# awsaf49/vip-cup-2022

Measured on AMD Instinct MI355X. Metric: images/sec (200x200, full ensemble), higher is better.
Workload: dtype f16; 1 GPU; ensemble8; precision=fast, distinct_images=5120, global_batch=256, parallelism=image-parallel dp1, one all-gather of scores, member_streams=3

## Files before the change

### include/vipcup_hip.h

```cpp
#ifndef VIPCUP_HIP_H
#define VIPCUP_HIP_H

#include <stddef.h>
#include <stdint.h>

#ifdef __cplusplus
extern "C" {
#endif

typedef enum vip_status {
    VIP_OK = 0,
    VIP_ERR_BAD_ARG = -1,
    VIP_ERR_ALIGNMENT = -2,
    VIP_ERR_UNSUPPORTED = -3,
    VIP_ERR_LAUNCH = -4,
    VIP_ERR_JPEG = -5,
    VIP_ERR_PNG = -6,
    VIP_ERR_WEBP = -7
} vip_status;

enum { VIP_ACT_NONE = 0, VIP_ACT_RELU = 1, VIP_ACT_SILU = 2, VIP_ACT_GELU = 3, VIP_ACT_SIGMOID = 4 };

int vip_version(void);
const char* vip_last_error(void);

typedef struct vip_conv_desc {
    int B, H, W;
    int Cin, Cout;
    int kh, kw, sh, sw;
    int pt, pl;
    int Ho, Wo;
    int groups;
    int ldx, cin_off;
    int ldy, cout_off;
    int ldr, res_off;
    int ldw;
    int act_pre, act_post;
} vip_conv_desc;

int vip_conv2d_nhwc_f16(const void* x, const void* w, const float* bias, const void* residual,
                        void* y, const vip_conv_desc* d, void* stream);

int vip_conv2d_gated_nhwc_f16(const void* x, const void* gate, const void* w, const float* bias, const void* residual,
                              void* y, const vip_conv_desc* d, void* stream);

int vip_conv2d_hilo_nhwc_f16(const void* x, const void* w_hi, const void* w_lo, const float* bias, const void* residual,
                             void* y, const vip_conv_desc* d, void* stream);

int vip_conv2d_out_gated_nhwc_f16(const void* x, const void* w, const void* w_lo, const float* bias, const void* out_gate,
                                  const void* residual, void* y, const vip_conv_desc* d, void* stream);
int vip_conv2d_out_gated_variant(const vip_conv_desc* d, int has_w_lo, char* variant, size_t cap);
int vip_conv2d_out_gated2_nhwc_f16(const void* x, const void* w, const void* w_lo, const float* bias, const void* out_gate,
                                   const void* residual, void* y, void* y2, int act2, const vip_conv_desc* d, void* stream);
int vip_conv2d_out_gated2_variant(const vip_conv_desc* d, int has_w_lo, int act2, char* variant, size_t cap);

int vip_gemm_bias_act_f16(const void* A, const void* W, const float* bias, const void* residual,
                          void* C, int M, int N, int K, int lda, int ldw, int ldc, int ldr,
                          int act_pre, int act_post, void* stream);

int vip_ln_gemm_supported(int M, int K, int N, int act);
int vip_ln_gemm_bias_act_f16(const void* A, const float* ln_gamma, const float* ln_beta, float ln_eps, const void* W,
                             const float* bias, const void* residual, void* C, int M, int N, int K, int lda, int ldw,
                             int ldc, int ldr, int act_pre, int act_post, void* stream);

int vip_gemm_split_f16(const void* A, const void* W, const float* bias, void* C, int M, int N, int K, int lda,
                       int ldw, int act, void* stream);

int vip_gemm_split2_f16(const void* A, const void* W, const float* bias, void* C, int M, int N, int K, int ldw, int act,
                        void* stream);
int vip_gemm_split2_hilo_f16(const void* A, const void* W, const void* W_lo, const float* bias, void* C, int M, int N, int K, int ldw,
                             int act, void* stream);

int vip_mlp_fused_supported(int M, int C, int hidden, int act);
int vip_mlp_fused_plan(int M, int C, int hidden, int act, int* workgroups, int* tile_rows);
int vip_mlp_fused_f16(const void* x, const float* ln_gamma, const float* ln_beta, float ln_eps, const void* w1,
                      const float* b1, const void* w2, const float* b2, const void* residual, void* y, int M, int C,
                      int hidden, int ldx, int ldw1, int ldw2, int ldy, int ldr, int act, void* stream);

int vip_se_gate_f16(const void* x, const void* w1, const float* b1, const void* w2, const float* b2, void* gate,
                    int B, int HW, int C, int ldx, int Cr, int ldw1, int Cout, int ldw2, int act1, int act2,
                    int split, void* stream);
int vip_se_gate_hilo_f16(const void* x, const void* w1, const void* w1_lo, const float* b1, const void* w2, const float* b2, void* gate,
                         int B, int HW, int C, int ldx, int Cr, int ldw1, int Cout, int ldw2, int act1, int act2, int split,
                         void* stream);

int vip_dwconv2d_nhwc_f16(const void* x, const float* w, const float* bias, void* y,
                          int B, int H, int W, int C, int k, int stride, int pt, int pl,
                          int Ho, int Wo, int act, void* stream);

int vip_dwconv2d_pool_parts(int B, int H, int W, int C, int k, int stride, int Ho, int Wo);
long vip_dwconv2d_tile_plan(int B, int H, int W, int C, int k, int stride, int Ho, int Wo, int pooled, int* workgroups, int* geom);
int vip_dwconv2d_pool_nhwc_f16(const void* x, const float* w, const float* bias, void* y, float* partials, int parts,
                               int B, int H, int W, int C, int k, int stride, int pt, int pl, int Ho, int Wo, int act,
                               void* stream);
int vip_se_gate_pooled_f16(const float* partials, int parts, const void* w1, const float* b1, const void* w2,
                           const float* b2, void* gate, int B, int HW, int C, int Cr, int ldw1, int Cout, int ldw2,
                           int act1, int act2, int split, void* stream);

int vip_layernorm_f16(const void* x, const float* gamma, const float* beta, void* y,
                      int rows, int C, float eps, void* stream);

int vip_pool2d_nhwc_f16(const void* x, void* y, int B, int H, int W, int C, int ldx, int ldy,
                        int k, int stride, int pt, int pl, int Ho, int Wo, int mode, void* stream);

int vip_global_avgpool_f16(const void* x, void* y, int B, int HW, int C, int ldx, void* stream);

int vip_global_avgpool_split_f16(const void* x, void* y, int B, int HW, int C, int ldx, void* stream);

int vip_gap_dense_f32(const void* x, const float* W, const float* bias, float* out, int B, int HW, int C,
                      int ldx, int N, void* stream);

int vip_gap_ln_dense_f32(const void* x, const float* gamma, const float* beta, float eps, const float* W, const float* bias,
                         float* out, int B, int HW, int C, int ldx, int N, void* stream);

int vip_scale_add_act_f16(const void* x, const void* scale, const void* residual, void* y,
                          int B, int HW, int C, int act, void* stream);
int vip_scale_add_act2_f16(const void* x, const void* scale, const void* residual, void* y, void* y2,
                           int B, int HW, int C, int act, int act2, void* stream);
int vip_scale_add_act3_f16(const void* x, const void* scale, int scale_planes, const void* residual, void* y, void* y2,
                           int B, int HW, int C, int act, int act2, void* stream);

int vip_mul_f16(const void* a, const void* b, void* y, long rows, int C, int lda, int a_off, int ldb, int b_off,
                int ldy, int y_off, void* stream);

int vip_radix_combine_f16(const void* x, const void* scale, void* y, int B, int HW, int C, int radix,
                          void* stream);
int vip_radix_combine2_f16(const void* x, const void* scale, int scale_planes, void* y, int B, int HW, int C, int radix,
                           void* stream);

int vip_gcvit_attn_block_supported(int C, int heads, int ws);
int vip_gcvit_attn_block_f16(const void* x, const void* q_global, const float* ln_gamma, const float* ln_beta, float ln_eps,
                             const void* wqkv, int ldwq, const float* bqkv, const void* wproj, int ldwp, const float* bproj,
                             const float* table, void* y, int B, int Hp, int Wp, int C, int heads, int ws, float scale,
                             void* stream);

int vip_window_attn_fwd_f16(const void* qkv, const void* q_global, const float* bias_table,
                            void* out, int B, int Hp, int Wp, int C, int heads, int ws, int nq,
                            float scale, void* stream);

int vip_mhsa_fwd_f16(const void* qkv, void* out, int B, int N, int D, int heads, float scale,
                     void* stream);

int vip_vit_tokens_f16(const void* patches, const void* cls_token, const void* pos_embed, void* out,
                       int B, int n_patches, int D, void* stream);

typedef struct vip_jpeg_desc {
// ... 357 lines not shown
```

### vip-cup-2022_amd/_abi.py

```python
import ctypes as C
import os

import torch

_HERE = os.path.dirname(os.path.abspath(__file__))
LIB_PATH = os.environ.get("VIP_LIB_PATH") or os.path.join(_HERE, "libvipcup_hip.so")

_lib = None


class VipError(RuntimeError):
    pass


class ConvDesc(C.Structure):
    _fields_ = [(n, C.c_int) for n in (
        "B", "H", "W", "Cin", "Cout", "kh", "kw", "sh", "sw", "pt", "pl", "Ho", "Wo", "groups",
        "ldx", "cin_off", "ldy", "cout_off", "ldr", "res_off", "ldw", "act_pre", "act_post")]


class JpegDesc(C.Structure):
    _fields_ = [("width", C.c_int32), ("height", C.c_int32), ("ncomp", C.c_int32),
                ("hsamp", C.c_int32 * 3), ("vsamp", C.c_int32 * 3),
                ("blocks_w", C.c_int32 * 3), ("blocks_h", C.c_int32 * 3),
                ("coef_off", C.c_int64 * 3), ("qt", (C.c_uint16 * 64) * 3), ("rgb_coded", C.c_int32)]


class PngDesc(C.Structure):
    _fields_ = [("width", C.c_int32), ("height", C.c_int32), ("bit_depth", C.c_int32), ("color_type", C.c_int32),
                ("interlace", C.c_int32), ("channels", C.c_int32), ("bpp", C.c_int32), ("palette_size", C.c_int32),
                ("stream_off", C.c_int64), ("pass_off", C.c_int64 * 7), ("pass_w", C.c_int32 * 7), ("pass_h", C.c_int32 * 7),
                ("palette", (C.c_uint8 * 3) * 256)]


class WebpDesc(C.Structure):
    _fields_ = [("width", C.c_int32), ("height", C.c_int32), ("has_alpha", C.c_int32), ("coded_width", C.c_int32),
                ("n_transforms", C.c_int32), ("stats", C.c_int32), ("type", C.c_int32 * 4), ("bits", C.c_int32 * 4),
                ("xsize", C.c_int32 * 4), ("stream_off", C.c_int64), ("data_off", C.c_int64 * 4), ("argb_off", C.c_int64)]


class Vp8Mb(C.Structure):
    _fields_ = [("ymode", C.c_uint8), ("uvmode", C.c_uint8), ("flevel", C.c_uint8), ("ilevel", C.c_uint8), ("hev", C.c_uint8),
                ("inner", C.c_uint8), ("segment", C.c_uint8), ("skip", C.c_uint8), ("bmodes", C.c_uint8 * 16), ("nz", C.c_uint32),
                ("dc_only", C.c_uint32), ("coef_idx", C.c_uint32), ("reserved", C.c_uint32)]


class Vp8Desc(C.Structure):
    _fields_ = [("width", C.c_int32), ("height", C.c_int32), ("mb_w", C.c_int32), ("mb_h", C.c_int32), ("has_alpha", C.c_int32),
                ("filter_type", C.c_int32), ("stats", C.c_int64), ("stream_off", C.c_int64), ("mb_off", C.c_int64),
                ("coef_off", C.c_int64), ("coef_blocks", C.c_int64), ("plane_off", C.c_int64)]


class Vp8EncParams(C.Structure):
    _fields_ = [("quality", C.c_int32), ("base_q", C.c_int32), ("y1", C.c_int32 * 2), ("y2", C.c_int32 * 2), ("uv", C.c_int32 * 2),
                ("filter_level", C.c_int32), ("flevel", C.c_int32), ("ilevel", C.c_int32), ("hev", C.c_int32), ("i4_bias", C.c_int32),
                ("reserved", C.c_int32), ("y1_inv", C.c_uint32 * 2), ("y2_inv", C.c_uint32 * 2), ("uv_inv", C.c_uint32 * 2)]


_vp, _i, _f, _sz = C.c_void_p, C.c_int, C.c_float, C.c_size_t

SIGNATURES = {
    "vip_version": (_i, []),
    "vip_last_error": (C.c_char_p, []),
    "vip_conv2d_nhwc_f16": (_i, [_vp, _vp, _vp, _vp, _vp, C.POINTER(ConvDesc), _vp]),
    "vip_conv2d_gated_nhwc_f16": (_i, [_vp, _vp, _vp, _vp, _vp, _vp, C.POINTER(ConvDesc), _vp]),
    "vip_conv2d_hilo_nhwc_f16": (_i, [_vp, _vp, _vp, _vp, _vp, _vp, C.POINTER(ConvDesc), _vp]),
    "vip_conv2d_out_gated_nhwc_f16": (_i, [_vp, _vp, _vp, _vp, _vp, _vp, _vp, C.POINTER(ConvDesc), _vp]),
    "vip_conv2d_out_gated_variant": (_i, [C.POINTER(ConvDesc), _i, C.c_char_p, _sz]),
    "vip_conv2d_out_gated2_nhwc_f16": (_i, [_vp, _vp, _vp, _vp, _vp, _vp, _vp, _vp, _i, C.POINTER(ConvDesc), _vp]),
    "vip_conv2d_out_gated2_variant": (_i, [C.POINTER(ConvDesc), _i, _i, C.c_char_p, _sz]),
    "vip_gemm_bias_act_f16": (_i, [_vp, _vp, _vp, _vp, _vp] + [_i] * 9 + [_vp]),
    "vip_ln_gemm_supported": (_i, [_i, _i, _i, _i]),
    "vip_ln_gemm_bias_act_f16": (_i, [_vp, _vp, _vp, _f] + [_vp] * 4 + [_i] * 9 + [_vp]),
    "vip_mlp_fused_supported": (_i, [_i, _i, _i, _i]),
    "vip_mlp_fused_plan": (_i, [_i] * 4 + [C.POINTER(_i)] * 2),
    "vip_mlp_fused_f16": (_i, [_vp, _vp, _vp, _f] + [_vp] * 6 + [_i] * 9 + [_vp]),
    "vip_se_gate_f16": (_i, [_vp] * 6 + [_i] * 11 + [_vp]),
    "vip_se_gate_hilo_f16": (_i, [_vp] * 7 + [_i] * 11 + [_vp]),
    "vip_gemm_split_f16": (_i, [_vp, _vp, _vp, _vp] + [_i] * 6 + [_vp]),
    "vip_gemm_split2_f16": (_i, [_vp, _vp, _vp, _vp] + [_i] * 5 + [_vp]),
    "vip_gemm_split2_hilo_f16": (_i, [_vp, _vp, _vp, _vp, _vp] + [_i] * 5 + [_vp]),
    "vip_dwconv2d_nhwc_f16": (_i, [_vp, _vp, _vp, _vp] + [_i] * 11 + [_vp]),
    "vip_dwconv2d_pool_parts": (_i, [_i] * 8),
    "vip_dwconv2d_tile_plan": (C.c_long, [_i] * 9 + [C.POINTER(_i)] * 2),
    "vip_dwconv2d_pool_nhwc_f16": (_i, [_vp, _vp, _vp, _vp, _vp] + [_i] * 12 + [_vp]),
    "vip_se_gate_pooled_f16": (_i, [_vp, _i] + [_vp] * 5 + [_i] * 10 + [_vp]),
    "vip_layernorm_f16": (_i, [_vp, _vp, _vp, _vp, _i, _i, _f, _vp]),
    "vip_pool2d_nhwc_f16": (_i, [_vp, _vp] + [_i] * 13 + [_vp]),
    "vip_global_avgpool_f16": (_i, [_vp, _vp, _i, _i, _i, _i, _vp]),
    "vip_global_avgpool_split_f16": (_i, [_vp, _vp, _i, _i, _i, _i, _vp]),
    "vip_gap_dense_f32": (_i, [_vp, _vp, _vp, _vp, _i, _i, _i, _i, _i, _vp]),
    "vip_experiments_built": (_i, []),
    "vip_gcvit_attn_block_supported": (_i, [_i, _i, _i]),
    "vip_gcvit_attn_block_f16": (_i, [_vp, _vp, _vp, _vp, _f, _vp, _i, _vp, _vp, _i, _vp, _vp, _vp] + [_i] * 6 + [_f, _vp]),
    "vip_mbconv_expand_dw_supported": (_i, [_i, _i, _i, _i]),
    "vip_mbconv_expand_dw_f16": (_i, [_vp] * 7 + [_i] * 14 + [_vp]),
    "vip_head_prob_f32": (_i, [_vp, _vp, _vp, _i, _i, _vp]),
    "vip_head_act_f32": (_i, [_vp, _vp, _i, _i, _i, _vp]),
    "vip_prob_to_score_f32": (_i, [_vp, _vp, _i, _i, _vp]),
    "vip_ensemble_mean_f32": (_i, [_vp, _vp, _i, _i, C.c_long, _vp]),
    "vip_gap_ln_dense_f32": (_i, [_vp, _vp, _vp, _f, _vp, _vp, _vp, _i, _i, _i, _i, _i, _vp]),
    "vip_scale_add_act_f16": (_i, [_vp, _vp, _vp, _vp, _i, _i, _i, _i, _vp]),
    "vip_scale_add_act2_f16": (_i, [_vp, _vp, _vp, _vp, _vp, _i, _i, _i, _i, _i, _vp]),
    "vip_scale_add_act3_f16": (_i, [_vp, _vp, _i, _vp, _vp, _vp, _i, _i, _i, _i, _i, _vp]),
    "vip_mul_f16": (_i, [_vp, _vp, _vp, C.c_long] + [_i] * 7 + [_vp]),
    "vip_radix_combine_f16": (_i, [_vp, _vp, _vp, _i, _i, _i, _i, _vp]),
    "vip_radix_combine2_f16": (_i, [_vp, _vp, _i, _vp, _i, _i, _i, _i, _vp]),
    "vip_window_attn_fwd_f16": (_i, [_vp, _vp, _vp, _vp] + [_i] * 7 + [_f, _vp]),
    "vip_mhsa_fwd_f16": (_i, [_vp, _vp, _i, _i, _i, _i, _f, _vp]),
    "vip_jpeg_probe_h": (_i, [_vp, _sz, _vp, _vp]),
    "vip_jpeg_entropy_decode_h": (_i, [_vp, _vp, _i, _vp, _vp, _sz, _vp, _i]),
    "vip_jpeg_idct_rgb_u8": (_i, [_vp, _vp, _i, _i, _vp, _vp, _i, _i, _vp]),
    "vip_jpeg_quality_tables_h": (_i, [_i, _vp, _vp]),
    "vip_jpeg_encode_layout_h": (_i, [_i, _i, _i, _i, _vp, _vp]),
    "vip_jpeg_fdct_quant_u8": (_i, [_vp, _vp, _i, _i, _vp, _vp, _i, _i, _vp]),
    "vip_resample_coeffs_h": (_i, [_i, _i, _i, _vp, _sz, _vp, _sz, _vp]),
    "vip_resample_tile_shape": (_i, [_vp, _vp, _vp]),
    "vip_resample_rgb_u8": (_i, [_vp, _vp, _i, _i, _vp, _vp, _i, _i, _vp, _vp, _i, _i, _i, _vp]),
    "vip_blur_weights_h": (_i, [C.c_double, _i, _vp, _sz]),
    "vip_blur_gauss_rgb_u8": (_i, [_vp, _vp, _i, _i, _vp, _i, _i, _vp, _i, _i, _vp]),
    "vip_median_rgb_u8": (_i, [_vp, _vp, _i, _i, _vp, _i, _i, _i, _i, _vp]),
    "vip_sharpen_rgb_u8": (_i, [_vp, _vp, _i, _i, _vp, _i, _i, _vp, _i, _i, _i, _i, _vp]),
    "vip_warp_affine_rgb_u8": (_i, [_vp, _vp, _i, _i, _vp, _vp, _i, _i, _vp, _i, _i, _vp]),
    "vip_colour_rgb_u8": (_i, [_vp, _vp, _i, _i, _vp, _i, _i, _vp, _vp, _vp, _i, _vp]),
    "vip_noise_rgb_u8": (_i, [_vp, _vp, _i, _i, _vp, _i, _i, _i, C.c_int64, C.c_uint32, _vp, _vp, _i, _vp]),
    "vip_noise_rgb_u8_placed": (_i, [_vp, _vp, _i, _i, _vp, _i, _i, _i, C.c_int64, C.c_uint32, _vp, _vp, _i, _i, _vp]),
    "vip_tone_hist_u8": (_i, [_vp, _vp, _i, _i, _i, _i, _i, _vp, _i, _vp]),
    "vip_tone_lut_u8": (_i, [_vp, _i, _i, _i, _i, _vp, _vp]),
    "vip_tone_apply_rgb_u8": (_i, [_vp, _vp, _i, _i, _vp, _i, _i, _vp, _i, _i, _i, _i, _vp]),
    "vip_tone_apply_rgb_u8_placed": (_i, [_vp, _vp, _i, _i, _vp, _i, _i, _vp, _i, _i, _i, _i, _i, _vp]),
    "vip_png_probe_h": (_i, [_vp, _sz, _vp, _vp]),
    "vip_png_inflate_h": (_i, [_vp, _vp, _i, _vp, _vp, _sz, _vp, _i]),
    "vip_png_unfilter_rgb_u8": (_i, [_vp, _vp, _i, _vp, _i, _i, _vp]),
    "vip_webp_probe_h": (_i, [_vp, _sz, _vp, _vp]),
    "vip_webp_entropy_h": (_i, [_vp, _vp, _i, _vp, _vp, _sz, _vp, _i]),
    "vip_webp_inverse_rgb_u8": (_i, [_vp, _vp, _i, _vp, _i, _i, _vp]),
    "vip_vp8_probe_h": (_i, [_vp, _sz, _vp, _vp]),
    "vip_vp8_entropy_h": (_i, [_vp, _vp, _i, _vp, _vp, _sz, _vp, _i]),
    "vip_vp8_scratch_bytes": (_i, [_vp, _i, _vp]),
    "vip_vp8_reconstruct_rgb_u8": (_i, [_vp, _sz, _vp, _i, _vp, _sz, _vp, _i, _i, _vp]),
    "vip_vp8_default_stages": (_i, []),
    "vip_vp8_reconstruct_stages_rgb_u8": (_i, [_vp, _sz, _vp, _i, _vp, _sz, _vp, _i, _i, _i, _vp]),
    "vip_vp8_encode_params_h": (_i, [_i, _vp]),
    "vip_vp8_encode_layout_h": (_i, [_vp, _i, _i, _vp, _vp, _vp]),
    "vip_vp8_encode_rgb_u8": (_i, [_vp, _vp, _i, _i, _i, _i, _vp, _sz, _vp, _sz, _vp, _sz, _vp]),
    "vip_bicubic_table_f32": (_i, [_vp]),
    "vip_resize_bicubic_norm_f16": (_i, [_vp, _vp, _vp, _i, _i, _i, _vp, _i, _i, _i, _vp]),
    "vip_tile_resize_bicubic_norm_f16": (_i, [_vp, _vp, _vp, _i, _i, _i, _i, _vp, _i, _i, _i, _vp]),
    "vip_tile_resize_bicubic_norm_s32": (_i, [_vp, _vp, _vp, _i, _i, _i, _i, _vp, _i, _i, _i, _vp]),
    "vip_tile_aggregate_f32": (_i, [_vp, _vp, _i, _i, _i, _f, _vp, _vp]),
    "vip_image_mean_u8": (_i, [_vp, _vp, _i, _i, _i, _vp, _vp]),
    "vip_occlude_resize_bicubic_norm_f16": (_i, [_vp] * 5 + [_i] * 4 + [_vp, _i, _i, _i, _vp]),
    "vip_occlude_resize_bicubic_norm_s32": (_i, [_vp] * 5 + [_i] * 4 + [_vp, _i, _i, _i, _vp]),
    "vip_occlusion_cells_f32": (_i, [_vp, _vp, _vp, _i, _i, _i, _i, _i, _f, _vp, _vp, _vp]),
    "vip_occlusion_map": (_i, [_vp, _vp, _i, _i, _i, _i, _vp, _i, _vp]),
    "vip_tta_augment_f16": (_i, [_vp, _vp, _vp, _i, _i, _i, _i, _vp]),
# ... 81 lines not shown
```

### vip-cup-2022_amd/csrc/conv_igemm.hip

```cpp
#include "common.hpp"
#include <stdlib.h>
#include <string.h>
#include <type_traits>

#ifndef VIP_GEMM_H2
#define VIP_GEMM_H2 0
#endif

#ifndef VIP_MFMA_PRIO
#define VIP_MFMA_PRIO 1
#endif
#ifndef VIP_MFMA_PRIO_TILE
#define VIP_MFMA_PRIO_TILE 1
#endif

namespace {

constexpr bool H2 = VIP_GEMM_H2;
__device__ __forceinline__ int h2_pos(int c) { return H2 ? (((c & 1) << 2) | (c >> 1)) : c; }
constexpr unsigned OOB2 = 0xFFFFFFE0u;
constexpr int ESZ = H2 ? 4 : 2;

struct ConvArgs {
    const f16* x;
    const f16* w;
    const float* bias;
    const f16* res;
    f16* y;
    int H, W, Ho, Wo;
    int Cin_g, Cout_g;
    int kh, kw, sh, sw, pt, pl;
    int ldx, ldy, ldr, ldw;
    int cin_off, cout_off, res_off;
    int M, K;
    long x_span_bytes;
    long y_span_bytes, res_span_bytes;
    int bias_elems;
    int act_pre, act_post;
    int m_blocks, n_blocks;
    const f16* w_lo;
    const f16* gate;
    int y_lo_off;
    int gate_hw;
    const f16* ogate;
    int ogate_elems;
    unsigned hw_magic;
    float out_scale;
    int* status;
    const float* ln_g;
    const float* ln_b;
    float ln_eps;
};

struct ConvArgs2 : ConvArgs {
    f16* y2;
};

enum Family { PW_GEMM, ROWS_GEMM, GEMM8P, PWX, PWK_DIRECT, PWK_GEMM, IM2COL, CONV_IGEMM };
struct Plan {
    Family family;
    int mode;
    int ng, pt, wn, ks, ksc, bm, bn;
    bool gated, hilo, ln, xsplit, pipe;
    bool pf2;
    int m_blocks, n_blocks;
    int n_chunks, nb_ch, lds_stride;
};

template <int... Vs, class F>
int with_const(int v, F&& f) {
    int st = VIP_ERR_UNSUPPORTED;
    if (!((v == Vs && ((st = f(std::integral_constant<int, Vs>{})), true)) || ...)) vip_set_error("vip_conv2d_nhwc_f16: no instantiation for %d", v);
    return st;
}

inline int device_cus() {
    static const int cus = [] {
        hipDeviceProp_t pr;
        int dev = 0;
        return (hipGetDevice(&dev) == hipSuccess && hipGetDeviceProperties(&pr, dev) == hipSuccess && pr.multiProcessorCount > 0)
                   ? pr.multiProcessorCount : 256;
    }();
    return cus;
}

template <int ACT, bool RES, int POST>
__device__ __forceinline__ void h2_store8(const ConvArgs& a, const f32x4& q0, const f32x4& q1, unsigned off, unsigned roff,
                                          const __amdgpu_buffer_rsrc_t& rb_res, const __amdgpu_buffer_rsrc_t& rb_y) {
    f32x2 p[4] = {{q0[0], q0[1]}, {q0[2], q0[3]}, {q1[0], q1[1]}, {q1[2], q1[3]}};
#pragma unroll
    for (int e = 0; e < 4; ++e) p[e] = vip_act2<ACT>(p[e] * a.out_scale);
    if constexpr (RES) {
        const uint4 rh = __builtin_bit_cast(uint4, __builtin_amdgcn_raw_buffer_load_b128(rb_res, roff, 0, 0));
        const uint4 rl = __builtin_bit_cast(uint4, __builtin_amdgcn_raw_buffer_load_b128(rb_res, roff + 16u, 0, 0));
        const unsigned rhw[4] = {rh.x, rh.y, rh.z, rh.w}, rlw[4] = {rl.x, rl.y, rl.z, rl.w};
#pragma unroll
        for (int e = 0; e < 4; ++e) {
            float px = p[e].x, py = p[e].y;
            asm("v_fma_mix_f32 %0, %1, 1.0, %0 op_sel_hi:[1,0,0]" : "+v"(px) : "v"(rhw[e]));
            asm("v_fma_mix_f32 %0, %1, 1.0, %0 op_sel:[1,0,0] op_sel_hi:[1,0,0]" : "+v"(py) : "v"(rhw[e]));
            asm("v_fma_mix_f32 %0, %1, 1.0, %0 op_sel_hi:[1,0,0]" : "+v"(px) : "v"(rlw[e]));
            asm("v_fma_mix_f32 %0, %1, 1.0, %0 op_sel:[1,0,0] op_sel_hi:[1,0,0]" : "+v"(py) : "v"(rlw[e]));
            p[e] = (f32x2){px, py};
        }
    }
    if constexpr (POST == 1) {
#pragma unroll
        for (int e = 0; e < 4; ++e) p[e] = (f32x2){fmaxf(p[e].x, 0.f), fmaxf(p[e].y, 0.f)};
    } else if constexpr (POST == 2) {
#pragma unroll
        for (int e = 0; e < 4; ++e) p[e] = (f32x2){vip_act_strict(p[e].x, a.act_post), vip_act_strict(p[e].y, a.act_post)};
    }
    typedef unsigned short u16x2 __attribute__((ext_vector_type(2)));
    unsigned hw[4], lw[4];
    u16x2 mx = {0, 0};
#pragma unroll
    for (int e = 0; e < 4; ++e) {
        hw[e] = __builtin_bit_cast(unsigned, __builtin_convertvector(p[e], f16x2));
        const float px = p[e].x, py = p[e].y;
        asm("v_fma_mixlo_f16 %0, %1, -1.0, %2 op_sel_hi:[1,0,0]" : "=v"(lw[e]) : "v"(hw[e]), "v"(px));
        asm("v_fma_mixhi_f16 %0, %1, -1.0, %2 op_sel:[1,0,0] op_sel_hi:[1,0,0]" : "+v"(lw[e]) : "v"(hw[e]), "v"(py));
        mx = __builtin_elementwise_max(mx, __builtin_bit_cast(u16x2, hw[e] & 0x7FFF7FFFu));
    }
    typedef __attribute__((__vector_size__(4 * sizeof(unsigned)))) unsigned u32x4;
    const u32x4 oh = {hw[0], hw[1], hw[2], hw[3]}, ol = {lw[0], lw[1], lw[2], lw[3]};
    __builtin_amdgcn_raw_buffer_store_b128(oh, rb_y, off, 0, 0);
    __builtin_amdgcn_raw_buffer_store_b128(ol, rb_y, off + 16u, 0, 0);
    if (a.status && off != OOB2 && (mx.x >= 0x7C00 || mx.y >= 0x7C00)) *a.status = VIP_H2_OVERFLOW;
}

__device__ __forceinline__ int swz_x(int row, int chunk) { return row * 128 + ((chunk ^ (row & 7)) << 4); }
__device__ __forceinline__ int swz_w(int row, int chunk) {
    const int key = (((row >> 3) & 3) << 1) | ((row >> 1) & 1);
    return row * 128 + ((chunk ^ key) << 4);
}

template <int ACT>
__device__ __forceinline__ float act_t(float v) {
    if constexpr (ACT == VIP_ACT_RELU) return v > 0.f ? v : 0.f;
    else if constexpr (ACT == VIP_ACT_SILU) return v * vip_sigmoid(v);
    else if constexpr (ACT == VIP_ACT_GELU) return 0.5f * v * (1.f + vip_erf(v * 0.70710678118654752f));
    else if constexpr (ACT == VIP_ACT_SIGMOID) return vip_sigmoid(v);
    else return v;
}

template <int MT, int ACT>
__device__ __forceinline__ void epilogue(const ConvArgs& a, f32x4 (&acc)[MT][4], int m_base, int n_first, int group) {
// ... 192 lines not shown
        const char* sb = sa + A_BYTES;
#pragma unroll
        for (int ks = 0; ks < 2; ++ks) {
            const int ch = ks * 4 + lq;
            U4H8 wf[4], xf[MT];
#pragma unroll
            for (int nt = 0; nt < 4; ++nt) wf[nt].u = *reinterpret_cast<const uint4*>(sb + swz_w(wrow_base + (nt >> 1) * 32 + (nt & 1) * 4, ch));
#pragma unroll
            for (int mt = 0; mt < MT; ++mt) xf[mt].u = *reinterpret_cast<const uint4*>(sa + swz_x(xrow_base + mt * 16, ch));
            if constexpr (H2) {
                U4H8 wl[4];
                if (ks == 0) {
#pragma unroll
                    for (int nt = 0; nt < 4; ++nt) wl[nt].u = *reinterpret_cast<const uint4*>(sb + swz_w(wrow_base + (nt >> 1) * 32 + (nt & 1) * 4, 4 + lq));
                } else {
#pragma unroll
                    for (int nt = 0; nt < 4; ++nt) wf[nt].u = *reinterpret_cast<const uint4*>(sb + swz_w(wrow_base + (nt >> 1) * 32 + (nt & 1) * 4, lq));
                }
                if (VIP_MFMA_PRIO_TILE) __builtin_amdgcn_s_setprio(1);
#pragma unroll
                for (int mt = 0; mt < MT; ++mt)
#pragma unroll
                    for (int nt = 0; nt < 4; ++nt) {
                        if (ks == 0) acc[mt][nt] = __builtin_amdgcn_mfma_f32_16x16x32_f16(wl[nt].h, xf[mt].h, acc[mt][nt], 0, 0, 0);
                        acc[mt][nt] = __builtin_amdgcn_mfma_f32_16x16x32_f16(wf[nt].h, xf[mt].h, acc[mt][nt], 0, 0, 0);
                    }
                if (VIP_MFMA_PRIO_TILE) __builtin_amdgcn_s_setprio(0);
                continue;
            }
            if (VIP_MFMA_PRIO_TILE) __builtin_amdgcn_s_setprio(1);
#pragma unroll
            for (int mt = 0; mt < MT; ++mt)
#pragma unroll
                for (int nt = 0; nt < 4; ++nt)
                    acc[mt][nt] = __builtin_amdgcn_mfma_f32_16x16x32_f16(wf[nt].h, xf[mt].h, acc[mt][nt], 0, 0, 0);
            if (VIP_MFMA_PRIO_TILE) __builtin_amdgcn_s_setprio(0);
        }
        if (kt + 1 < nk) store_tiles(buf ^ 1);
        __syncthreads();
    }

    const int m_base = m0 + wave_m0 + l15;
    const int n_first = n0 + wave_n0 + lq * 8;
    switch (a.act_pre) {
        case VIP_ACT_RELU: epilogue<MT, VIP_ACT_RELU>(a, acc, m_base, n_first, group); break;
        case VIP_ACT_SILU: epilogue<MT, VIP_ACT_SILU>(a, acc, m_base, n_first, group); break;
        case VIP_ACT_GELU: epilogue<MT, VIP_ACT_GELU>(a, acc, m_base, n_first, group); break;
        case VIP_ACT_SIGMOID: epilogue<MT, VIP_ACT_SIGMOID>(a, acc, m_base, n_first, group); break;
        default: epilogue<MT, VIP_ACT_NONE>(a, acc, m_base, n_first, group); break;
    }
}

struct GateLds {
    const float* g;
    int img0, stride, n0;
};

__device__ __forceinline__ unsigned image_of(const ConvArgs& a, unsigned m) {
    unsigned img = __umulhi(m, a.hw_magic);
    if (m - img * (unsigned)a.gate_hw >= (unsigned)a.gate_hw) ++img;
    return img;
}

__device__ __forceinline__ int stage_out_gate(const ConvArgs& a, float* g_lds, int stride, int m_first, int rows, int n0, int nch, int t,
                                              int nthreads) {
    const __amdgpu_buffer_rsrc_t rb_g = __builtin_amdgcn_make_buffer_rsrc((void*)a.ogate, 0, (unsigned)a.ogate_elems * 2u, 0x00020000);
    const int img0 = (int)image_of(a, (unsigned)min(m_first, a.M - 1)), img1 = (int)image_of(a, (unsigned)min(m_first + rows - 1, a.M - 1));
    const int q = nch >> 2;
    for (int i = t; i < (img1 - img0 + 1) * q; i += nthreads) {
        const int im = i / q, c = (i - im * q) * 4, n = n0 + c;
        const unsigned off = n < a.Cout_g ? ((unsigned)(img0 + im) * 2u * (unsigned)a.Cout_g + (unsigned)n) * 2u : 0xFFFFFFF0u;
        typedef __attribute__((__vector_size__(2 * sizeof(unsigned)))) unsigned u32x2;
        const u32x2 hv = __builtin_amdgcn_raw_buffer_load_b64(rb_g, off, 0, 0);
        const u32x2 lv = __builtin_amdgcn_raw_buffer_load_b64(rb_g, n < a.Cout_g ? off + (unsigned)a.Cout_g * 2u : 0xFFFFFFF0u, 0, 0);
        const f16x4 hh = __builtin_bit_cast(f16x4, hv), ll = __builtin_bit_cast(f16x4, lv);
        f32x4 gv;
#pragma unroll
        for (int j = 0; j < 4; ++j) gv[j] = (float)hh[j] + (float)ll[j];
        *reinterpret_cast<f32x4*>(g_lds + im * stride + c) = gv;
    }
    return img0;
}

template <int PT, int ACT, bool RES, bool POST_RELU, bool OGATE = false, bool Y2 = false>
__device__ __forceinline__ void pw_epilogue(const ConvArgs& a, f32x4 (&acc)[PT][4], int m_base, int n_first,
                                            const __amdgpu_buffer_rsrc_t& rb_res, const __amdgpu_buffer_rsrc_t& rb_y, GateLds gl = GateLds{},
                                            const __amdgpu_buffer_rsrc_t* rb_y2 = nullptr) {
    constexpr unsigned OOB = 0xFFFFFFF0u;
    if constexpr (H2) {
#pragma unroll
        for (int p = 0; p < PT; ++p) {
            const int m = m_base + p * 16;
#pragma unroll
            for (int h = 0; h < 2; ++h) {
                const int n = n_first + h * 32;
                const bool ok = (m < a.M) & (n < a.Cout_g);
                const unsigned off = ok ? (unsigned)(((long)m * a.ldy + a.cout_off + n) * 4) : OOB2;
                const unsigned roff = (RES && ok) ? (unsigned)(((long)m * a.ldr + a.res_off + n) * 4) : OOB2;
                h2_store8<ACT, RES, POST_RELU ? 1 : 0>(a, acc[p][h * 2], acc[p][h * 2 + 1], off, roff, rb_res, rb_y);
            }
        }
        return;
    }
    static_assert(!(OGATE && H2), "the output gate is carried by the fp16-storage build only");
    static_assert(OGATE || !Y2, "the second output belongs to the output-gated epilogue");
#pragma unroll
    for (int p = 0; p < PT; ++p) {
        const int m = m_base + p * 16;
        int g_row = 0;
        if constexpr (OGATE) g_row = m < a.M ? ((int)image_of(a, (unsigned)m) - gl.img0) * gl.stride - gl.n0 : -gl.n0;
#pragma unroll
        for (int h = 0; h < 2; ++h) {
            const int n = n_first + h * 32;
            const bool ok = (m < a.M) & (n < a.Cout_g);
            U4H8 r;
            f32x4 g0, g1;
            if constexpr (RES)
                r.u = __builtin_bit_cast(uint4, __builtin_amdgcn_raw_buffer_load_b128(
                                                    rb_res, ok ? ((unsigned)m * (unsigned)a.ldr + (unsigned)(a.res_off + n)) * 2u : OOB, 0, 0));
            if constexpr (OGATE) {
                g0 = *reinterpret_cast<const f32x4*>(gl.g + g_row + n);
                g1 = *reinterpret_cast<const f32x4*>(gl.g + g_row + n + 4);
            }
            U4H8 o;
#pragma unroll
            for (int j = 0; j < 8; j += 2) {
                const f32x4 av = acc[p][h * 2 + (j >> 2)];
                f32x2 t = vip_act2<ACT>((f32x2){av[j & 3], av[(j & 3) + 1]});
                if constexpr (OGATE) {
                    const f32x4 gq = j < 4 ? g0 : g1;
                    t = t * (f32x2){gq[j & 3], gq[(j & 3) + 1]};
                }
                if constexpr (RES) t = t + (f32x2){(float)r.e[j], (float)r.e[j + 1]};
                if constexpr (POST_RELU) t = (f32x2){fmaxf(t.x, 0.f), fmaxf(t.y, 0.f)};
                o.e[j] = (f16)t.x;
                o.e[j + 1] = (f16)t.y;
            }
            __builtin_amdgcn_raw_buffer_store_b128(
                __builtin_bit_cast(__attribute__((__vector_size__(4 * sizeof(unsigned)))) unsigned, o.u), rb_y,
                ok ? ((unsigned)m * (unsigned)a.ldy + (unsigned)(a.cout_off + n)) * 2u : OOB, 0, 0);
            if constexpr (Y2) {
                U4H8 o2;
#pragma unroll
                for (int j = 0; j < 8; ++j) o2.e[j] = (f16)vip_act((float)o.e[j], VIP_ACT_SILU);
                __builtin_amdgcn_raw_buffer_store_b128(
                    __builtin_bit_cast(__attribute__((__vector_size__(4 * sizeof(unsigned)))) unsigned, o2.u), *rb_y2,
                    ok ? ((unsigned)m * (unsigned)a.ldy + (unsigned)(a.cout_off + n)) * 2u : OOB, 0, 0);
            }
        }
    }
}

template <int KS, int PT, bool PRE, bool HILO, bool OG = false, bool Y2 = false>
__global__ __launch_bounds__(256, 2) void pw_gemm_kernel(std::conditional_t<Y2, ConvArgs2, ConvArgs> a, int nb_ch, int lds_stride, int n_tiles,
                                                         int mode) {
    static_assert(OG || !Y2, "the second output belongs to the output-gated instantiations");
    extern __shared__ __attribute__((aligned(16))) char smem[];
    const int tid = threadIdx.x, lane = tid & 63, wave = tid >> 6;
    const int l15 = lane & 15, lq = lane >> 4;
    const int n_chunk0 = blockIdx.y * nb_ch;
    const int nch = min(nb_ch, ((a.Cout_g - n_chunk0) + 63) & ~63);
    constexpr unsigned OOB = 0xFFFFFFF0u;
    float* bias_lds = reinterpret_cast<float*>(smem + nb_ch * lds_stride);
    constexpr int OG_IMAGES = 4;
    float* g_lds = bias_lds + nb_ch + (tid >> 6) * (OG_IMAGES * nb_ch);

    {
        const __amdgpu_buffer_rsrc_t rw = __builtin_amdgcn_make_buffer_rsrc(
            (void*)a.w, 0, (unsigned)min((long)0xFFFFFFF0L, 2L * a.Cout_g * a.ldw), 0x00020000);
        const __amdgpu_buffer_rsrc_t rwl = __builtin_amdgcn_make_buffer_rsrc(
            (void*)a.w_lo, 0, HILO ? (unsigned)min((long)0xFFFFFFF0L, 2L * a.Cout_g * a.ldw) : 0u, 0x00020000);
        const int cpr = KS * 4;
        constexpr int HALVES = HILO ? 2 : 1;
        for (int i = tid; i < nch * cpr * HALVES; i += 256) {
            const int j = i / (cpr * HALVES), c2 = i - j * (cpr * HALVES);
            const int c = c2 < cpr ? c2 : c2 - cpr;
            const int t = (j >> 4) & 3, r = j & 15;
            const int ch = n_chunk0 + (j & ~63) + (t >> 1) * 32 + (r >> 2) * 8 + (t & 1) * 4 + (r & 3);
            const bool ok = (ch < a.Cout_g) & (c * 8 < a.K);
            const unsigned off = ok ? (unsigned)((ch * a.ldw + c * 8) * 2) : OOB;
            const uint4 v = __builtin_bit_cast(uint4, c2 < cpr ? __builtin_amdgcn_raw_buffer_load_b128(rw, off, 0, 0)
                                                               : __builtin_amdgcn_raw_buffer_load_b128(rwl, off, 0, 0));
            *reinterpret_cast<uint4*>(smem + j * lds_stride + (H2 ? ((c2 & ~7) | h2_pos(c2 & 7)) : c2) * 16) = v;
        }
        const __amdgpu_buffer_rsrc_t rb = __builtin_amdgcn_make_buffer_rsrc(
            (void*)a.bias, 0, a.bias ? (unsigned)(a.bias_elems * 4) : 0u, 0x00020000);
        for (int i = tid; i < nch; i += 256) {
            const int ch = n_chunk0 + i;
            bias_lds[i] = __builtin_bit_cast(float, __builtin_amdgcn_raw_buffer_load_b32(rb, ch < a.Cout_g ? (unsigned)(ch * 4) : OOB, 0, 0));
        }
    }
    __syncthreads();

    const __amdgpu_buffer_rsrc_t rx = __builtin_amdgcn_make_buffer_rsrc(
        (void*)(a.x + a.cin_off), 0, (unsigned)min((long)0xFFFFFFF0L, a.x_span_bytes - 2L * a.cin_off), 0x00020000);
    const __amdgpu_buffer_rsrc_t rb_res =
        __builtin_amdgcn_make_buffer_rsrc((void*)a.res, 0, a.res ? (unsigned)a.res_span_bytes : 0u, 0x00020000);
    const __amdgpu_buffer_rsrc_t rb_y = __builtin_amdgcn_make_buffer_rsrc((void*)a.y, 0, (unsigned)a.y_span_bytes, 0x00020000);
    const char* wl = smem + l15 * lds_stride + lq * 16;

    auto load_x = [&](int tile, U4H8 (&xf)[KS][PT]) {
        const int m0 = tile * (64 * PT) + wave * (16 * PT);
#pragma unroll
        for (int ks = 0; ks < KS; ++ks)
#pragma unroll
            for (int p = 0; p < PT; ++p) {
                const int m = m0 + p * 16 + l15, k = H2 ? (ks >> 1) * 64 + lq * 16 + (ks & 1) * 8 : ks * 32 + lq * 8;
                const bool ok = (m < a.M) & (k < a.K);
                xf[ks][p].u = __builtin_bit_cast(
                    uint4, __builtin_amdgcn_raw_buffer_load_b128(rx, ok ? (unsigned)((m * a.ldx + k) * 2) : OOB, 0, 0));
            }
// ... 56 lines not shown
                for (int p = 0; p < PT; ++p)
#pragma unroll
                    for (int nt = 0; nt < 4; ++nt)
                        acc[p][nt] = __builtin_amdgcn_mfma_f32_16x16x32_f16(wf[nt].h, xf[ks][p].h, ks == 0 ? bv[nt] : acc[p][nt], 0, 0, 0);
                if constexpr (HILO) {
#pragma unroll
                    for (int nt = 0; nt < 4; ++nt) wf[nt].u = *reinterpret_cast<const uint4*>(ws + nt * 16 * lds_stride + (KS + ks) * 64);
#pragma unroll
                    for (int p = 0; p < PT; ++p)
#pragma unroll
                        for (int nt = 0; nt < 4; ++nt)
                            acc[p][nt] = __builtin_amdgcn_mfma_f32_16x16x32_f16(wf[nt].h, xf[ks][p].h, acc[p][nt], 0, 0, 0);
                }
            }
            const int m_base = m0 + l15, n_first = n_chunk0 + sub + lq * 8;
            if constexpr (Y2) {
                const __amdgpu_buffer_rsrc_t rb_y2 = __builtin_amdgcn_make_buffer_rsrc((void*)a.y2, 0, (unsigned)a.y_span_bytes, 0x00020000);
                if (mode == 8) pw_epilogue<PT, VIP_ACT_NONE, true, true, true, true>(a, acc, m_base, n_first, rb_res, rb_y, gl, &rb_y2);
                else pw_epilogue<PT, VIP_ACT_NONE, true, false, true, true>(a, acc, m_base, n_first, rb_res, rb_y, gl, &rb_y2);
            } else if constexpr (OG) {
                if (mode == 8) pw_epilogue<PT, VIP_ACT_NONE, true, true, true>(a, acc, m_base, n_first, rb_res, rb_y, gl);
                else pw_epilogue<PT, VIP_ACT_NONE, true, false, true>(a, acc, m_base, n_first, rb_res, rb_y, gl);
            } else
            switch (mode) {
                case 1: pw_epilogue<PT, VIP_ACT_RELU, false, false>(a, acc, m_base, n_first, rb_res, rb_y); break;
                case 2: pw_epilogue<PT, VIP_ACT_SILU, false, false>(a, acc, m_base, n_first, rb_res, rb_y); break;
                case 3: pw_epilogue<PT, VIP_ACT_GELU, false, false>(a, acc, m_base, n_first, rb_res, rb_y); break;
                case 4: pw_epilogue<PT, VIP_ACT_SIGMOID, false, false>(a, acc, m_base, n_first, rb_res, rb_y); break;
                case 5: pw_epilogue<PT, VIP_ACT_NONE, true, false>(a, acc, m_base, n_first, rb_res, rb_y); break;
                case 6: pw_epilogue<PT, VIP_ACT_NONE, true, true>(a, acc, m_base, n_first, rb_res, rb_y); break;
                default: pw_epilogue<PT, VIP_ACT_NONE, false, false>(a, acc, m_base, n_first, rb_res, rb_y); break;
            }
        }
        if constexpr (PRE) {
#pragma unroll
            for (int ks = 0; ks < KS; ++ks)
#pragma unroll
                for (int p = 0; p < PT; ++p) xf[ks][p] = xn[ks][p];
        } else {
            if (tile + (int)gridDim.x < n_tiles) load_x(tile + gridDim.x, xf);
        }
    }
}

constexpr size_t pw_og_lds(int nb_ch) { return (size_t)4 * 4 * nb_ch * 4; }

template <int KS, int PT, bool HILO, bool OG = false>
int launch_pw(const ConvArgs& a, const Plan& p, hipStream_t s) {
    constexpr bool PRE = OG ? KS <= 2 : KS <= 3;
    const int n_tiles = (a.M + 64 * PT - 1) / (64 * PT);
    int gx = (2 * device_cus() + p.n_chunks - 1) / p.n_chunks;
    if (gx > n_tiles) gx = n_tiles;
    static bool attr_set = false;
    if (!attr_set) {
        (void)hipFuncSetAttribute(reinterpret_cast<const void*>(pw_gemm_kernel<KS, PT, PRE, HILO, OG>),
                                  hipFuncAttributeMaxDynamicSharedMemorySize, 160 * 1024);
        attr_set = true;
    }
    hipLaunchKernelGGL((pw_gemm_kernel<KS, PT, PRE, HILO, OG>), dim3((unsigned)gx, (unsigned)p.n_chunks), dim3(256),
                       (size_t)p.nb_ch * (p.lds_stride + 4) + (OG ? pw_og_lds(p.nb_ch) : 0), s, a, p.nb_ch, p.lds_stride, n_tiles, p.mode);
    return vip_launch_status("vip_conv2d_nhwc_f16(pw)");
}

template <int KS, int PT, bool HILO>
int launch_pw_og2(const ConvArgs& a, const Plan& p, f16* y2, hipStream_t s) {
    constexpr bool PRE = KS <= 2;
    const int n_tiles = (a.M + 64 * PT - 1) / (64 * PT);
    int gx = (2 * device_cus() + p.n_chunks - 1) / p.n_chunks;
    if (gx > n_tiles) gx = n_tiles;
    static bool attr_set = false;
    if (!attr_set) {
        (void)hipFuncSetAttribute(reinterpret_cast<const void*>(pw_gemm_kernel<KS, PT, PRE, HILO, true, true>),
                                  hipFuncAttributeMaxDynamicSharedMemorySize, 160 * 1024);
        attr_set = true;
    }
    ConvArgs2 a2;
    static_cast<ConvArgs&>(a2) = a;
    a2.y2 = y2;
    hipLaunchKernelGGL((pw_gemm_kernel<KS, PT, PRE, HILO, true, true>), dim3((unsigned)gx, (unsigned)p.n_chunks), dim3(256),
                       (size_t)p.nb_ch * (p.lds_stride + 4) + pw_og_lds(p.nb_ch), s, a2, p.nb_ch, p.lds_stride, n_tiles, p.mode);
    return vip_launch_status("vip_conv2d_out_gated2_nhwc_f16(pw)");
}

template <int NG, bool GATED, int PT = 4, bool OG2 = false>
__global__ __launch_bounds__(256, 2) void pwk_direct_kernel(std::conditional_t<OG2, ConvArgs2, ConvArgs> a, int mode) {
    static_assert(!(OG2 && (GATED || H2)), "the second output: fp16 storage, no input gate");
    constexpr int NB = 64 * NG, ROWB = 160;
    constexpr int STAGE = NB * ROWB;
    constexpr int W_IT = NB / 32;
    __shared__ __attribute__((aligned(16))) char smem[2 * STAGE];
    const int tid = threadIdx.x, lane = tid & 63, wave = tid >> 6;
    const int l15 = lane & 15, lq = lane >> 4;
    constexpr unsigned OOB = 0xFFFFFFF0u;

    int bid = blockIdx.x;
    {
        const int nwg = gridDim.x;
        const int q = nwg >> 3, r = nwg & 7;
        const int xcd = bid & 7, idx = bid >> 3;
        bid = (xcd < r ? xcd * (q + 1) : r * (q + 1) + (xcd - r) * q) + idx;
    }
    const int mb = bid / a.n_blocks, nb = bid - mb * a.n_blocks;
    const int m0 = mb * (64 * PT) + wave * (16 * PT);
    const int n0 = nb * NB;

    const __amdgpu_buffer_rsrc_t rw = __builtin_amdgcn_make_buffer_rsrc(
        (void*)a.w, 0, (unsigned)min((long)0xFFFFFFF0L, 2L * a.Cout_g * a.ldw), 0x00020000);
    const __amdgpu_buffer_rsrc_t rx = __builtin_amdgcn_make_buffer_rsrc(
        (void*)(a.x + a.cin_off), 0, (unsigned)min((long)0xFFFFFFF0L, a.x_span_bytes - 2L * a.cin_off), 0x00020000);
    const __amdgpu_buffer_rsrc_t rb_res =
        __builtin_amdgcn_make_buffer_rsrc((void*)a.res, 0, a.res ? (unsigned)a.res_span_bytes : 0u, 0x00020000);
    const __amdgpu_buffer_rsrc_t rb_y = __builtin_amdgcn_make_buffer_rsrc((void*)a.y, 0, (unsigned)a.y_span_bytes, 0x00020000);
    const __amdgpu_buffer_rsrc_t rb_bias =
        __builtin_amdgcn_make_buffer_rsrc((void*)a.bias, 0, a.bias ? (unsigned)(a.bias_elems * 4) : 0u, 0x00020000);

    const int wc = tid & 7;
    unsigned w_off[W_IT];
    int w_lds[W_IT];
#pragma unroll
    for (int i = 0; i < W_IT; ++i) {
        const int j = (tid >> 3) + 32 * i;
        const int t = (j >> 4) & 3, r = j & 15;
        const int ch = n0 + (j & ~63) + (t >> 1) * 32 + (r >> 2) * 8 + (t & 1) * 4 + (r & 3);
        w_off[i] = ch < a.Cout_g ? (unsigned)((ch * a.ldw + wc * 8) * 2) : OOB;
        w_lds[i] = j * ROWB + h2_pos(wc) * 16;
    }
    unsigned x_off[PT];
#pragma unroll
    for (int p = 0; p < PT; ++p) {
        const int m = m0 + p * 16 + l15;
        x_off[p] = m < a.M ? (unsigned)((m * a.ldx + lq * (H2 ? 16 : 8)) * 2) : 0xFFFF0000u;
    }
    const __amdgpu_buffer_rsrc_t rg = __builtin_amdgcn_make_buffer_rsrc(
        (void*)a.gate, 0, GATED ? (unsigned)min((long)0xFFFFFFF0L, (H2 ? 2L : 4L) * ((a.M + a.gate_hw - 1) / a.gate_hw) * a.K) : 0u, 0x00020000);
    unsigned g_off[PT];
#pragma unroll
    for (int p = 0; p < PT; ++p) {
        const int m = m0 + p * 16 + l15;
        g_off[p] = (GATED && m < a.M) ? (H2 ? (unsigned)((m / a.gate_hw) * a.K * 2 + lq * 32) : (unsigned)(((m / a.gate_hw) * 2 * a.K + lq * 8) * 2))
                                      : 0xFFFF0000u;
    }
    const int nk = (a.K + 63) >> 6;

    uint4 wst[W_IT];
    auto load_w = [&](int kc) {
        const bool ok = kc * 64 + wc * 8 < a.K;
#pragma unroll
        for (int i = 0; i < W_IT; ++i)
            wst[i] = __builtin_bit_cast(uint4, __builtin_amdgcn_raw_buffer_load_b128(rw, ok ? w_off[i] + kc * 128 : OOB, 0, 0));
    };
    auto store_w = [&](int buf) {
#pragma unroll
        for (int i = 0; i < W_IT; ++i) *reinterpret_cast<uint4*>(smem + buf * STAGE + w_lds[i]) = wst[i];
    };
    U4H8 xf[2][PT], gq[GATED ? 2 : 1][GATED ? PT : 1];
    auto load_x = [&](int kc, int ks) {
        const bool ok = kc * 64 + (H2 ? lq * 16 + ks * 8 : ks * 32 + lq * 8) < a.K;
#pragma unroll
        for (int p = 0; p < PT; ++p)
            xf[ks][p].u = __builtin_bit_cast(
                uint4, __builtin_amdgcn_raw_buffer_load_b128(rx, ok ? x_off[p] + kc * 128 + ks * (H2 ? 16 : 64) : OOB, 0, 0));
    };
    auto load_g = [&](int kc, int ks) {
        if constexpr (GATED && H2) {
            const bool ok = kc * 64 + lq * 16 < a.K;
#pragma unroll
            for (int p = 0; p < PT; ++p) {
                gq[0][p].u = __builtin_bit_cast(uint4, __builtin_amdgcn_raw_buffer_load_b128(rg, ok ? g_off[p] + kc * 128 : OOB, 0, 0));
                gq[1][p].u = __builtin_bit_cast(uint4, __builtin_amdgcn_raw_buffer_load_b128(rg, ok ? g_off[p] + kc * 128 + 16 : OOB, 0, 0));
            }
        } else if constexpr (GATED) {
            const bool ok = kc * 64 + ks * 32 + lq * 8 < a.K;
#pragma unroll
            for (int p = 0; p < PT; ++p) {
                gq[0][p].u = __builtin_bit_cast(
                    uint4, __builtin_amdgcn_raw_buffer_load_b128(rg, ok ? g_off[p] + kc * 128 + ks * 64 : OOB, 0, 0));
                gq[1][p].u = __builtin_bit_cast(
                    uint4, __builtin_amdgcn_raw_buffer_load_b128(rg, ok ? g_off[p] + kc * 128 + ks * 64 + 2 * a.K : OOB, 0, 0));
            }
        }
    };
    auto gate_x = [&](int ks) {
        if constexpr (GATED && H2) {
#pragma unroll
            for (int p = 0; p < PT; ++p) {
                float xv[8], gv[8];
                h2_join8(xf[0][p], xf[1][p], xv);
                h2_join8(gq[0][p], gq[1][p], gv);
#pragma unroll
                for (int j = 0; j < 8; ++j) xv[j] *= gv[j];
                h2_split8(xv, xf[0][p], xf[1][p]);
            }
        } else if constexpr (GATED) {
#pragma unroll
            for (int p = 0; p < PT; ++p)
                xf[ks][p].h = __builtin_elementwise_fma(xf[ks][p].h, gq[0][p].h, xf[ks][p].h * gq[1][p].h);
        }
    };

    f32x4 acc[NG][PT][4];
    {
#pragma unroll
        for (int g = 0; g < NG; ++g)
#pragma unroll
            for (int nt = 0; nt < 4; ++nt) {
                const int n = n0 + g * 64 + (nt >> 1) * 32 + lq * 8 + (nt & 1) * 4;
                const f32x4 bv = __builtin_bit_cast(
                    f32x4, __builtin_amdgcn_raw_buffer_load_b128(rb_bias, n < a.Cout_g ? (unsigned)(n * 4) : OOB, 0, 0));
#pragma unroll
                for (int p = 0; p < PT; ++p) acc[g][p][nt] = bv;
            }
    }

    load_w(0);
    load_x(0, 0);
    load_x(0, 1);
    load_g(0, 0);
    store_w(0);
    __syncthreads();

    auto compute = [&](int buf, int ks) {
        const char* ws = smem + buf * STAGE + l15 * ROWB + lq * 16 + ks * 64;
#pragma unroll
        for (int g = 0; g < NG; ++g) {
            U4H8 wf[4];
            if constexpr (H2) {
                const char* wh = ws - ks * 64;
                U4H8 wl[4];
#pragma unroll
                for (int nt = 0; nt < 4; ++nt) wf[nt].u = *reinterpret_cast<const uint4*>(wh + (g * 64 + nt * 16) * ROWB);
                if (ks == 0) {
#pragma unroll
                    for (int nt = 0; nt < 4; ++nt) wl[nt].u = *reinterpret_cast<const uint4*>(wh + 64 + (g * 64 + nt * 16) * ROWB);
                }
                if (VIP_MFMA_PRIO) __builtin_amdgcn_s_setprio(1);
#pragma unroll
                for (int nt = 0; nt < 4; ++nt)
#pragma unroll
                    for (int p = 0; p < PT; ++p) {
                        if (ks == 0) acc[g][p][nt] = __builtin_amdgcn_mfma_f32_16x16x32_f16(wl[nt].h, xf[0][p].h, acc[g][p][nt], 0, 0, 0);
                        acc[g][p][nt] = __builtin_amdgcn_mfma_f32_16x16x32_f16(wf[nt].h, xf[ks][p].h, acc[g][p][nt], 0, 0, 0);
                    }
                if (VIP_MFMA_PRIO) __builtin_amdgcn_s_setprio(0);
                continue;
            }
#pragma unroll
            for (int nt = 0; nt < 4; ++nt) wf[nt].u = *reinterpret_cast<const uint4*>(ws + (g * 64 + nt * 16) * ROWB);
            if (VIP_MFMA_PRIO) __builtin_amdgcn_s_setprio(1);
#pragma unroll
            for (int nt = 0; nt < 4; ++nt)
#pragma unroll
                for (int p = 0; p < PT; ++p)
                    acc[g][p][nt] = __builtin_amdgcn_mfma_f32_16x16x32_f16(wf[nt].h, xf[ks][p].h, acc[g][p][nt], 0, 0, 0);
            if (VIP_MFMA_PRIO) __builtin_amdgcn_s_setprio(0);
        }
    };

    for (int kc = 0; kc < nk; ++kc) {
        const int buf = kc & 1;
        load_w(kc + 1);
        __builtin_amdgcn_sched_barrier(0);
        if constexpr (GATED && H2) {
            gate_x(0);
            __builtin_amdgcn_sched_barrier(0);
            load_g(kc + 1, 0);
            __builtin_amdgcn_sched_barrier(0);
        } else if constexpr (GATED) {
            gate_x(0);
            __builtin_amdgcn_sched_barrier(0);
            load_g(kc, 1);
            __builtin_amdgcn_sched_barrier(0);
        }
        compute(buf, 0);
        __builtin_amdgcn_sched_barrier(0);
        load_x(kc + 1, 0);
        __builtin_amdgcn_sched_barrier(0);
        if constexpr (GATED && !H2) {
            gate_x(1);
            __builtin_amdgcn_sched_barrier(0);
            load_g(kc + 1, 0);
            __builtin_amdgcn_sched_barrier(0);
        }
        compute(buf, 1);
        __builtin_amdgcn_sched_barrier(0);
        load_x(kc + 1, 1);
        store_w(buf ^ 1);
        __syncthreads();
    }

    int m_base = m0 + l15, n_lane = n0 + lq * 8;
    asm volatile("" : "+v"(m_base), "+v"(n_lane));
    GateLds gl{};
#if !VIP_GEMM_H2
    if constexpr (!GATED) {
        if (mode >= 7) {
            float* g_lds = reinterpret_cast<float*>(smem);
            const int img0 = stage_out_gate(a, g_lds, NB, mb * (64 * PT), 64 * PT, n0, NB, (int)threadIdx.x, 256);
            __syncthreads();
            gl = GateLds{g_lds, img0, NB, n0};
        }
    }
#endif
    auto epi = [&](auto gtag) {
        constexpr int G_ = decltype(gtag)::value;
        const int n_first = n_lane + G_ * 64;
#if !VIP_GEMM_H2
        if constexpr (OG2) {
            const __amdgpu_buffer_rsrc_t rb_y2 = __builtin_amdgcn_make_buffer_rsrc((void*)a.y2, 0, (unsigned)a.y_span_bytes, 0x00020000);
            if (mode == 8) pw_epilogue<PT, VIP_ACT_NONE, true, true, true, true>(a, acc[G_], m_base, n_first, rb_res, rb_y, gl, &rb_y2);
            else pw_epilogue<PT, VIP_ACT_NONE, true, false, true, true>(a, acc[G_], m_base, n_first, rb_res, rb_y, gl, &rb_y2);
            return;
        }
#endif
        switch (mode) {
            case 1: pw_epilogue<PT, VIP_ACT_RELU, false, false>(a, acc[G_], m_base, n_first, rb_res, rb_y); break;
            case 2: pw_epilogue<PT, VIP_ACT_SILU, false, false>(a, acc[G_], m_base, n_first, rb_res, rb_y); break;
            case 3: pw_epilogue<PT, VIP_ACT_GELU, false, false>(a, acc[G_], m_base, n_first, rb_res, rb_y); break;
            case 4: pw_epilogue<PT, VIP_ACT_SIGMOID, false, false>(a, acc[G_], m_base, n_first, rb_res, rb_y); break;
            case 5: pw_epilogue<PT, VIP_ACT_NONE, true, false>(a, acc[G_], m_base, n_first, rb_res, rb_y); break;
            case 6: pw_epilogue<PT, VIP_ACT_NONE, true, true>(a, acc[G_], m_base, n_first, rb_res, rb_y); break;
#if !VIP_GEMM_H2
            case 7: if constexpr (!GATED) pw_epilogue<PT, VIP_ACT_NONE, true, false, true>(a, acc[G_], m_base, n_first, rb_res, rb_y, gl); break;
            case 8: if constexpr (!GATED) pw_epilogue<PT, VIP_ACT_NONE, true, true, true>(a, acc[G_], m_base, n_first, rb_res, rb_y, gl); break;
#endif
            default: pw_epilogue<PT, VIP_ACT_NONE, false, false>(a, acc[G_], m_base, n_first, rb_res, rb_y); break;
        }
    };
    epi(std::integral_constant<int, 0>{});
    if constexpr (NG > 1) epi(std::integral_constant<int, 1>{});
}


template <int KSC, int PT, bool LN>
__device__ __forceinline__ void pwx_body(const ConvArgs& a, int mode) {
    constexpr int NG = 2, NB = 64 * NG, ROWB = 160;
    constexpr int STAGE = NB * ROWB;
    constexpr int W_IT = NB / 32;
    __shared__ __attribute__((aligned(16))) char smem[2 * STAGE];
    const int tid = threadIdx.x, lane = tid & 63, wave = tid >> 6;
    const int l15 = lane & 15, lq = lane >> 4;
    constexpr unsigned OOB = 0xFFFFFFF0u;

    int bid = blockIdx.x;
    {
        const int nwg = gridDim.x;
        const int q = nwg >> 3, r = nwg & 7;
        const int xcd = bid & 7, idx = bid >> 3;
        bid = (xcd < r ? xcd * (q + 1) : r * (q + 1) + (xcd - r) * q) + idx;
    }
    const int m0 = bid * (64 * PT) + wave * (16 * PT);

    const __amdgpu_buffer_rsrc_t rw = __builtin_amdgcn_make_buffer_rsrc(
        (void*)a.w, 0, (unsigned)min((long)0xFFFFFFF0L, 2L * a.Cout_g * a.ldw), 0x00020000);
    const __amdgpu_buffer_rsrc_t rx = __builtin_amdgcn_make_buffer_rsrc(
        (void*)(a.x + a.cin_off), 0, (unsigned)min((long)0xFFFFFFF0L, a.x_span_bytes - 2L * a.cin_off), 0x00020000);
    const __amdgpu_buffer_rsrc_t rb_res =
        __builtin_amdgcn_make_buffer_rsrc((void*)a.res, 0, a.res ? (unsigned)a.res_span_bytes : 0u, 0x00020000);
    const __amdgpu_buffer_rsrc_t rb_y = __builtin_amdgcn_make_buffer_rsrc((void*)a.y, 0, (unsigned)a.y_span_bytes, 0x00020000);
    const __amdgpu_buffer_rsrc_t rb_bias =
        __builtin_amdgcn_make_buffer_rsrc((void*)a.bias, 0, a.bias ? (unsigned)(a.bias_elems * 4) : 0u, 0x00020000);

    const int wc = tid & 7;
    int w_ch[W_IT], w_lds[W_IT];
#pragma unroll
    for (int i = 0; i < W_IT; ++i) {
        const int j = (tid >> 3) + 32 * i;
        const int t = (j >> 4) & 3, r = j & 15;
        w_ch[i] = (j & ~63) + (t >> 1) * 32 + (r >> 2) * 8 + (t & 1) * 4 + (r & 3);
        w_lds[i] = j * ROWB + h2_pos(wc) * 16;
    }
    uint4 wst[W_IT];
    auto load_w = [&](int n0, int kc) {
        const bool okk = kc * 64 + wc * 8 < a.K;
#pragma unroll
        for (int i = 0; i < W_IT; ++i) {
            const int ch = n0 + w_ch[i];
            wst[i] = __builtin_bit_cast(uint4, __builtin_amdgcn_raw_buffer_load_b128(
                                                   rw, (okk && ch < a.Cout_g) ? (unsigned)((ch * a.ldw + wc * 8) * 2) + kc * 128 : OOB, 0, 0));
        }
    };
    auto store_w = [&](int buf) {
#pragma unroll
        for (int i = 0; i < W_IT; ++i) *reinterpret_cast<uint4*>(smem + buf * STAGE + w_lds[i]) = wst[i];
    };

    U4H8 xf[2 * KSC][PT];
#pragma unroll
    for (int p = 0; p < PT; ++p) {
        const int m = m0 + p * 16 + l15;
        const unsigned xo = m < a.M ? ((unsigned)m * (unsigned)a.ldx + (unsigned)(lq * (H2 ? 16 : 8))) * 2u : 0xFFFF0000u;
#pragma unroll
        for (int kc = 0; kc < KSC; ++kc)
#pragma unroll
            for (int ks = 0; ks < 2; ++ks) {
                const bool ok = kc * 64 + (H2 ? lq * 16 + ks * 8 : ks * 32 + lq * 8) < a.K;
                xf[2 * kc + ks][p].u = __builtin_bit_cast(
                    uint4, __builtin_amdgcn_raw_buffer_load_b128(rx, ok ? xo + kc * 128 + ks * (H2 ? 16 : 64) : OOB, 0, 0));
            }
    }
    if constexpr (LN && !H2) {
        __shared__ __attribute__((aligned(16))) float lnp[2][64 * KSC];
        for (int c = tid; c < 64 * KSC; c += 256) {
            lnp[0][c] = c < a.K ? a.ln_g[c] : 0.f;
            lnp[1][c] = c < a.K ? a.ln_b[c] : 0.f;
        }
        __syncthreads();
        const float fk = (float)a.K;
        float mean[PT], rstd[PT];
        auto pin = [&]() {
#pragma unroll
            for (int i = 0; i < 2 * KSC; ++i)
#pragma unroll
                for (int p = 0; p < PT; ++p) {
// ... 455 lines not shown
    load_w(0);
    load_x(0);
    store_w(0);
    store_x();
    __syncthreads();

    auto compute = [&](int buf, int ks) {
        const char* ws = smem + buf * STAGE + (WN > 1 ? wn * NB * ROWB : 0) + l15 * ROWB + lq * 16 + ks * 64;
        const char* xl = xs + l15 * ROWB + lq * 16 + ks * 64;
        U4H8 xf[PT];
#pragma unroll
        for (int p = 0; p < PT; ++p) xf[p].u = *reinterpret_cast<const uint4*>(xl + p * 16 * ROWB);
#pragma unroll
        for (int g = 0; g < NG; ++g) {
            U4H8 wf[4];
            if constexpr (H2) {
                const char* wh = ws - ks * 64;
                U4H8 wl[4];
#pragma unroll
                for (int nt = 0; nt < 4; ++nt) wf[nt].u = *reinterpret_cast<const uint4*>(wh + (g * 64 + nt * 16) * ROWB);
                if (ks == 0) {
#pragma unroll
                    for (int nt = 0; nt < 4; ++nt) wl[nt].u = *reinterpret_cast<const uint4*>(wh + 64 + (g * 64 + nt * 16) * ROWB);
                }
                if (VIP_MFMA_PRIO) __builtin_amdgcn_s_setprio(1);
#pragma unroll
                for (int nt = 0; nt < 4; ++nt)
#pragma unroll
                    for (int p = 0; p < PT; ++p) {
                        if (ks == 0) acc[g][p][nt] = __builtin_amdgcn_mfma_f32_16x16x32_f16(wl[nt].h, xf[p].h, acc[g][p][nt], 0, 0, 0);
                        acc[g][p][nt] = __builtin_amdgcn_mfma_f32_16x16x32_f16(wf[nt].h, xf[p].h, acc[g][p][nt], 0, 0, 0);
                    }
                if (VIP_MFMA_PRIO) __builtin_amdgcn_s_setprio(0);
                continue;
            }
#pragma unroll
            for (int nt = 0; nt < 4; ++nt) wf[nt].u = *reinterpret_cast<const uint4*>(ws + (g * 64 + nt * 16) * ROWB);
            if (VIP_MFMA_PRIO) __builtin_amdgcn_s_setprio(1);
#pragma unroll
            for (int nt = 0; nt < 4; ++nt)
#pragma unroll
                for (int p = 0; p < PT; ++p)
                    acc[g][p][nt] = __builtin_amdgcn_mfma_f32_16x16x32_f16(wf[nt].h, xf[p].h, acc[g][p][nt], 0, 0, 0);
            if (VIP_MFMA_PRIO) __builtin_amdgcn_s_setprio(0);
        }
    };

    for (int kc = 0; kc < nk; ++kc) {
        const int buf = kc & 1;
        load_w(kc + 1);
        load_x(kc + 1);
        __builtin_amdgcn_sched_barrier(0);
        compute(buf, 0);
        compute(buf, 1);
        __builtin_amdgcn_sched_barrier(0);
        store_w(buf ^ 1);
        if constexpr (WN > 1) __syncthreads();
        store_x();
        __syncthreads();
    }

    int m_base = m0 + l15, n_lane = n0 + lq * 8;
    asm volatile("" : "+v"(m_base), "+v"(n_lane));
    auto epi = [&](auto gtag) {
        constexpr int G_ = decltype(gtag)::value;
        const int n_first = n_lane + G_ * 64;
        switch (mode) {
            case 1: pw_epilogue<PT, VIP_ACT_RELU, false, false>(a, acc[G_], m_base, n_first, rb_res, rb_y); break;
            case 2: pw_epilogue<PT, VIP_ACT_SILU, false, false>(a, acc[G_], m_base, n_first, rb_res, rb_y); break;
            case 3: pw_epilogue<PT, VIP_ACT_GELU, false, false>(a, acc[G_], m_base, n_first, rb_res, rb_y); break;
            case 4: pw_epilogue<PT, VIP_ACT_SIGMOID, false, false>(a, acc[G_], m_base, n_first, rb_res, rb_y); break;
            case 5: pw_epilogue<PT, VIP_ACT_NONE, true, false>(a, acc[G_], m_base, n_first, rb_res, rb_y); break;
            case 6: pw_epilogue<PT, VIP_ACT_NONE, true, true>(a, acc[G_], m_base, n_first, rb_res, rb_y); break;
            default: pw_epilogue<PT, VIP_ACT_NONE, false, false>(a, acc[G_], m_base, n_first, rb_res, rb_y); break;
        }
    };
    epi(std::integral_constant<int, 0>{});
    if constexpr (NG > 1) epi(std::integral_constant<int, 1>{});
}

template <int NG>
int launch_pwk_direct(const ConvArgs& a, const Plan& p, hipStream_t s) {
    auto go = [&](auto kernel) { hipLaunchKernelGGL(kernel, dim3((unsigned)(a.m_blocks * a.n_blocks)), dim3(256), 0, s, a, p.mode); };
    if (p.pt == 1) p.gated ? go(pwk_direct_kernel<NG, true, 1>) : go(pwk_direct_kernel<NG, false, 1>);
#if VIP_BUILD_EXPERIMENTS
    else if (p.pf2) go(pwk_direct2_kernel<NG>);
#endif
    else p.gated ? go(pwk_direct_kernel<NG, true, 4>) : go(pwk_direct_kernel<NG, false, 4>);
    return vip_launch_status("vip_conv2d_nhwc_f16(pwk-direct)");
}

#if !VIP_GEMM_H2
template <int NG>
int launch_pwk_direct_og2(const ConvArgs& a, const Plan& p, f16* y2, hipStream_t s) {
    ConvArgs2 a2;
    static_cast<ConvArgs&>(a2) = a;
    a2.y2 = y2;
    auto go = [&](auto kernel) { hipLaunchKernelGGL(kernel, dim3((unsigned)(a.m_blocks * a.n_blocks)), dim3(256), 0, s, a2, p.mode); };
    if (p.pt == 1) go(pwk_direct_kernel<NG, false, 1, true>);
    else go(pwk_direct_kernel<NG, false, 4, true>);
    return vip_launch_status("vip_conv2d_out_gated2_nhwc_f16(pwk-direct)");
}
#endif

template <int NG, int WN, bool IM2COL>
int launch_pwk(const ConvArgs& a, int mode, int groups, hipStream_t s) {
    constexpr size_t smem = (2 * 64 * NG * WN + 4 * 64) * 160;
    static bool attr_set = false;
    if (!attr_set) {
        (void)hipFuncSetAttribute(reinterpret_cast<const void*>(pwk_gemm_kernel<NG, WN, IM2COL>),
                                  hipFuncAttributeMaxDynamicSharedMemorySize, (int)smem);
        attr_set = true;
    }
    const dim3 grid((unsigned)(a.m_blocks * a.n_blocks), (unsigned)groups);
    hipLaunchKernelGGL((pwk_gemm_kernel<NG, WN, IM2COL>), grid, dim3(256 * WN), smem, s, a, mode);
    return vip_launch_status(IM2COL ? "vip_conv2d_nhwc_f16(pwk-im2col)" : "vip_conv2d_nhwc_f16(pwk)");
}

#include "gemm8p.hpp"

template <bool XSPLIT, bool WLO = false>
__global__ __launch_bounds__(256) void rows_gemm_kernel(ConvArgs a) {
    constexpr unsigned OOB = 0xFFFFFFF0u;
    __shared__ float red[3][1][16][64];
    const int tid = threadIdx.x, lane = tid & 63, wave = tid >> 6;
    const int mw = 0, kq = wave;
    const int l15 = lane & 15, lq = lane >> 4;
    const int n0 = blockIdx.x * 16;
    const int m0 = blockIdx.y * 64;
    const __amdgpu_buffer_rsrc_t rw = __builtin_amdgcn_make_buffer_rsrc(
        (void*)a.w, 0, (unsigned)min((long)0xFFFFFFF0L, 2L * a.Cout_g * a.ldw), 0x00020000);
    const __amdgpu_buffer_rsrc_t rx = __builtin_amdgcn_make_buffer_rsrc(
        (void*)(a.x + a.cin_off), 0, (unsigned)min((long)0xFFFFFFF0L, a.x_span_bytes - 2L * a.cin_off), 0x00020000);
    const unsigned w_off = (n0 + l15 < a.Cout_g) ? (unsigned)(((n0 + l15) * a.ldw + lq * (H2 ? 16 : 8)) * 2) : 0xFFFF0000u;
    unsigned x_off[4];
#pragma unroll
    for (int p = 0; p < 4; ++p) {
        const int m = m0 + p * 16 + l15;
        x_off[p] = m < a.M ? (unsigned)((m * a.ldx + lq * (H2 ? 16 : 8)) * 2) : 0xFFFF0000u;
    }
    f32x4 acc[4];
#pragma unroll
    for (int p = 0; p < 4; ++p) acc[p] = (f32x4){0.f, 0.f, 0.f, 0.f};
    const int nks = H2 ? 2 * ((a.K + 63) >> 6) : (a.K + 31) >> 5;
    const int per = ((nks + 3) / 4 + 3) & ~3;
    const int ks_lo = kq * per, ks_hi = min(nks, ks_lo + per);
    if (m0 < a.M) {
        for (int ks0 = ks_lo; ks0 < ks_hi; ks0 += 4) {
            U4H8 wf[4], xf[4][4];
#pragma unroll
            for (int u = 0; u < 4; ++u) {
                const int kst = ks0 + u;
                const bool ok = (kst < ks_hi) & ((H2 ? (kst >> 1) * 64 + lq * 16 + (kst & 1) * 8 : kst * 32 + lq * 8) < a.K);
                const unsigned kb = H2 ? (unsigned)((kst >> 1) * 128 + (kst & 1) * 16) : (unsigned)(kst * 64);
                wf[u].u = __builtin_bit_cast(uint4, __builtin_amdgcn_raw_buffer_load_b128(rw, ok ? w_off + kb : OOB, 0, 0));
#pragma unroll
                for (int p = 0; p < 4; ++p)
                    xf[u][p].u = __builtin_bit_cast(uint4, __builtin_amdgcn_raw_buffer_load_b128(rx, ok ? x_off[p] + kb : OOB, 0, 0));
            }
            if constexpr (H2) {
#pragma unroll
                for (int u = 0; u < 4; u += 2)
#pragma unroll
                    for (int p = 0; p < 4; ++p) {
                        acc[p] = __builtin_amdgcn_mfma_f32_16x16x32_f16(wf[u + 1].h, xf[u][p].h, acc[p], 0, 0, 0);
                        acc[p] = __builtin_amdgcn_mfma_f32_16x16x32_f16(wf[u].h, xf[u + 1][p].h, acc[p], 0, 0, 0);
// ... 220 lines not shown
            const int pwx_on = pwx_env ? atoi(pwx_env) : 0;
            if (pwx_on && !gate && cout_g >= 256 && a.K <= (H2 ? 512 : 256) && a.K > 64 && M >= 16384 && a.x_span_bytes < 0xFFFF0000L - 2L * a.K) {
                const int ksc = (a.K + 63) >> 6;
                if (H2) {
                    if (ksc <= 4) return plan_pwx(p, a, 4, 2, false);
                    return plan_pwx(p, a, ksc <= 6 ? 6 : 8, 1, false);
                }
                return plan_pwx(p, a, ksc <= 2 ? 2 : ksc <= 3 ? 3 : 4, 2, false);
            }
            if ((a.K < xl_min_k || gate) && a.x_span_bytes < 0xFFFF0000L - 2L * a.K) return plan_pwk_direct(p, a);
            VIP_REQUIRE(!gate, VIP_ERR_UNSUPPORTED, "vip_conv2d_gated_nhwc_f16: input tensor too large (4 GB - 2K)");
            if (cout_g <= 64) return plan_pwk(p, a, 1, 1);
            static const int wn2_min_k = getenv("VIP_PWK_WN2K") ? atoi(getenv("VIP_PWK_WN2K")) : 1024;
            if (cout_g % 256 == 0 && a.K >= wn2_min_k && (long)((M + 255) / 256) * (cout_g / 256) >= 256) return plan_pwk(p, a, 2, 2);
            return plan_pwk(p, a, 2, 1);
        }
    }
    {
        static const int im2col_all = getenv("VIP_PWK_CONV") ? atoi(getenv("VIP_PWK_CONV")) : 0;
        if ((cin_g <= 16 || im2col_all > 0 || (im2col_all == 0 && M >= 32768)) && mode >= 0 && !gate && a.x_span_bytes < 0xFFFFFFF0L && d->H < 30000 &&
            d->W < 30000 && d->pt < 16 && d->pl < 16) {
            p.family = IM2COL; p.ng = cout_g <= 64 ? 1 : 2;
            plan_blocks(p, a, 256, 64 * p.ng);
            return VIP_OK;
        }
    }
    VIP_REQUIRE(!w_lo, VIP_ERR_UNSUPPORTED, "vip_conv2d_hilo_nhwc_f16: only 1x1 stride-1 ungrouped convolutions with K <= 256");
    VIP_REQUIRE(!gate, VIP_ERR_UNSUPPORTED,
                "vip_conv2d_gated_nhwc_f16: only 1x1 stride-1 ungrouped convolutions with (activation) or (residual [+ReLU]) "
                "epilogues take a gate; apply vip_scale_add_act_f16 first");
    p.family = CONV_IGEMM; p.bm = short_k ? 64 : 128; p.bn = cout_g <= 64 ? 64 : 128;
    plan_blocks(p, a, p.bm, p.bn);
    return VIP_OK;
}

static int launch(const Plan& p, ConvArgs a, int groups, hipStream_t s, f16* y2 = nullptr) {
    a.m_blocks = p.m_blocks; a.n_blocks = p.n_blocks;
#if !VIP_GEMM_H2
    if (y2) {
        if (p.mode < 7) return (int)VIP_ERR_UNSUPPORTED;
        if (p.family == PW_GEMM)
            return with_const<1, 2, 3, 4>(p.ks, [&](auto ks) {
                constexpr int KS = decltype(ks)::value;
                return p.hilo ? launch_pw_og2<KS, 4, true>(a, p, y2, s) : launch_pw_og2<KS, 4, false>(a, p, y2, s);
            });
        if (p.family == PWK_DIRECT) return p.ng == 1 ? launch_pwk_direct_og2<1>(a, p, y2, s) : launch_pwk_direct_og2<2>(a, p, y2, s);
        return (int)VIP_ERR_UNSUPPORTED;
    }
#endif
    switch (p.family) {
        case PW_GEMM:
            return with_const<1, 2, 3, 4, 6, 8>(p.ks, [&](auto ks) {
                constexpr int KS = decltype(ks)::value;
                if constexpr (!H2 && KS <= 4)
                    if (p.mode >= 7) return p.hilo ? launch_pw<KS, 4, true, true>(a, p, s) : launch_pw<KS, 4, false, true>(a, p, s);
                if (p.mode >= 7) return (int)VIP_ERR_UNSUPPORTED;
                return p.hilo ? launch_pw<KS, 4, true>(a, p, s) : launch_pw<KS, 4, false>(a, p, s);
            });
        case ROWS_GEMM:
            if constexpr (!H2)
                if (p.hilo) return launch_rows<true, true>(a, s);
            return p.xsplit ? launch_rows<true>(a, s) : launch_rows<false>(a, s);
        case GEMM8P: return launch_gemm8p(a, p.mode, p.pipe, s);
        case PWX:
#if !VIP_GEMM_H2
            if (p.ln) return with_const<2, 3, 4, 6>(p.ksc, [&](auto ksc) { return launch_pwx<decltype(ksc)::value, 2, true>(a, p.mode, s); });
#endif
            if (p.pt == 2) return with_const<2, 3, 4>(p.ksc, [&](auto ksc) { return launch_pwx<decltype(ksc)::value, 2, false>(a, p.mode, s); });
            return with_const<6, 8>(p.ksc, [&](auto ksc) { return launch_pwx<decltype(ksc)::value, 1, false>(a, p.mode, s); });
        case PWK_DIRECT: return p.ng == 1 ? launch_pwk_direct<1>(a, p, s) : launch_pwk_direct<2>(a, p, s);
        case PWK_GEMM:
            if (p.ng == 1) return launch_pwk<1, 1, false>(a, p.mode, groups, s);
            return p.wn == 1 ? launch_pwk<2, 1, false>(a, p.mode, groups, s) : launch_pwk<2, 2, false>(a, p.mode, groups, s);
        case IM2COL: return p.ng == 1 ? launch_pwk<1, 1, true>(a, p.mode, groups, s) : launch_pwk<2, 1, true>(a, p.mode, groups, s);
        case CONV_IGEMM:
            if (p.bn == 64) return p.bm == 64 ? launch_igemm<64, 64>(a, groups, s) : launch_igemm<128, 64>(a, groups, s);
            return p.bm == 64 ? launch_igemm<64, 128>(a, groups, s) : launch_igemm<128, 128>(a, groups, s);
    }
    return VIP_ERR_UNSUPPORTED;
}

static int conv2d_plan(const void* x, const void* gate, int y_lo_off, const void* w, const float* bias, const void* residual, void* y,
                       const vip_conv_desc* d, const void* w_lo, bool x_split, float out_scale, int* status, const float* ln_g,
                       const float* ln_b, float ln_eps, ConvArgs* args, Plan* p, const void* out_gate = nullptr) {
    VIP_REQUIRE(x && w && y && d, VIP_ERR_BAD_ARG, "vip_conv2d_nhwc_f16: null pointer");
    VIP_REQUIRE(d->B > 0 && d->H > 0 && d->W > 0 && d->Cin > 0 && d->Cout > 0 && d->kh > 0 && d->kw > 0 &&
                    d->sh > 0 && d->sw > 0 && d->Ho > 0 && d->Wo > 0 && d->groups > 0 && d->pt >= 0 && d->pl >= 0,
                VIP_ERR_BAD_ARG, "vip_conv2d_nhwc_f16: non-positive dimension");
    VIP_REQUIRE(d->Cin % d->groups == 0 && d->Cout % d->groups == 0, VIP_ERR_BAD_ARG,
                "vip_conv2d_nhwc_f16: channels (%d,%d) not divisible by groups %d", d->Cin, d->Cout, d->groups);
    const int cin_g = d->Cin / d->groups, cout_g = d->Cout / d->groups;
    VIP_REQUIRE(cin_g % 8 == 0 && cout_g % 8 == 0, VIP_ERR_ALIGNMENT,
                "vip_conv2d_nhwc_f16: Cin/groups=%d and Cout/groups=%d must be multiples of 8", cin_g, cout_g);
    VIP_REQUIRE(d->ldx % 8 == 0 && d->ldy % 8 == 0 && d->ldw % 8 == 0 && d->cin_off % 8 == 0 &&
                    d->cout_off % 8 == 0 && (!residual || (d->ldr % 8 == 0 && d->res_off % 8 == 0)),
                VIP_ERR_ALIGNMENT, "vip_conv2d_nhwc_f16: strides/offsets must be multiples of 8 halfs");
    constexpr int IN = H2 ? 2 : 1;
    VIP_REQUIRE(d->ldx >= d->cin_off + d->Cin && d->ldy >= d->cout_off + d->Cout && d->ldw >= IN * d->kh * d->kw * cin_g,
                VIP_ERR_BAD_ARG, "vip_conv2d_nhwc_f16: leading dimension smaller than the channel extent");
    VIP_REQUIRE(!H2 || (d->ldw % 16 == 0 && !w_lo && !y_lo_off && !x_split), VIP_ERR_BAD_ARG,
                "vip_conv2d_nhwc_h2: ldw must be a multiple of 16 halfs; no split variants");
    VIP_REQUIRE((unsigned)d->act_pre <= 4u && (unsigned)d->act_post <= 4u, VIP_ERR_BAD_ARG,
                "vip_conv2d_nhwc_f16: unknown activation code");
    const long M = (long)d->B * d->Ho * d->Wo;
    VIP_REQUIRE(M < (1L << 31) - 256, VIP_ERR_UNSUPPORTED, "vip_conv2d_nhwc_f16: B*Ho*Wo too large");

    ConvArgs& a = *args;
    a.x = (const f16*)x; a.w = (const f16*)w; a.bias = bias; a.res = (const f16*)residual; a.y = (f16*)y;
    a.H = d->H; a.W = d->W; a.Ho = d->Ho; a.Wo = d->Wo;
    a.Cin_g = cin_g * IN; a.Cout_g = cout_g;
    a.kh = d->kh; a.kw = d->kw; a.sh = d->sh; a.sw = d->sw; a.pt = d->pt; a.pl = d->pl;
    a.ldx = d->ldx * IN; a.ldy = d->ldy; a.ldr = d->ldr; a.ldw = d->ldw;
    a.cin_off = d->cin_off * IN; a.cout_off = d->cout_off; a.res_off = d->res_off;
    a.M = (int)M; a.K = d->kh * d->kw * cin_g * IN;
    a.x_span_bytes = 2L * IN * d->B * d->H * d->W * d->ldx;
    a.y_span_bytes = (long)ESZ * M * d->ldy;
    a.res_span_bytes = (long)ESZ * M * d->ldr;
    a.bias_elems = d->Cout;
    a.out_scale = out_scale;
    a.status = status;
    VIP_REQUIRE(a.y_span_bytes < 0xFFFFFFE0L && a.res_span_bytes < 0xFFFFFFE0L, VIP_ERR_UNSUPPORTED,
                "vip_conv2d_nhwc_f16: output or residual tensor exceeds the 4 GiB buffer-addressing range");
    VIP_REQUIRE(a.x_span_bytes < 0xFFFFFFF0L && 2L * d->Cout * d->ldw < 0xFFFFFFF0L, VIP_ERR_UNSUPPORTED,
                "vip_conv2d_nhwc_f16: input or weight tensor exceeds the 4 GiB buffer-addressing range");
    a.act_pre = d->act_pre; a.act_post = d->act_post;
    a.m_blocks = a.n_blocks = 0;
    a.w_lo = (const f16*)w_lo;
    a.gate = (const f16*)gate;
    a.gate_hw = d->Ho * d->Wo;
    a.y_lo_off = y_lo_off;
    a.ln_g = ln_g; a.ln_b = ln_b; a.ln_eps = ln_eps;
    a.ogate = (const f16*)out_gate;
    a.ogate_elems = 0;
    a.hw_magic = a.gate_hw > 1 ? (unsigned)((1L << 32) / a.gate_hw) : 0xFFFFFFFFu;
    if (!out_gate) return plan(a, d, x_split, p);
    VIP_REQUIRE(!H2 && residual && !gate && !y_lo_off && !x_split && !ln_g && d->groups == 1 && d->cout_off == 0 && d->act_pre == VIP_ACT_NONE &&
                    (d->act_post == VIP_ACT_NONE || d->act_post == VIP_ACT_RELU) && 4L * d->B * d->Cout < 0xFFFFFFF0L,
                VIP_ERR_UNSUPPORTED, "vip_conv2d_out_gated_nhwc_f16: ungrouped, residual [+ReLU] epilogue, no input gate, cout_off = 0");
    a.ogate_elems = 2 * d->B * d->Cout;
    const int st = plan(a, d, x_split, p);
    if (st != VIP_OK) return st;
    const bool pw_ok = p->family == PW_GEMM && p->ks <= 4 && 63 / a.gate_hw + 2 <= 4 &&
                       (size_t)p->nb_ch * (p->lds_stride + 4) + pw_og_lds(p->nb_ch) <= 80 * 1024;
    const bool pwk_ok = p->family == PWK_DIRECT && !p->gated && !p->pf2 && (64 * p->pt - 1) / a.gate_hw + 2 <= 80;
    VIP_REQUIRE((p->mode == 5 || p->mode == 6) && (pw_ok || pwk_ok), VIP_ERR_UNSUPPORTED,
                "vip_conv2d_out_gated_nhwc_f16: this shape's kernel carries no output gate (pw_gemm_kernel up to K = 128 and "
                "pwk_direct_kernel do)");
    p->mode += 2;
    return VIP_OK;
}

static int conv2d_impl(const void* x, const void* gate, int y_lo_off, const void* w, const float* bias, const void* residual, void* y,
                       const vip_conv_desc* d, void* stream, const void* w_lo = nullptr, bool x_split = false, float out_scale = 1.f,
                       int* status = nullptr, const float* ln_g = nullptr, const float* ln_b = nullptr, float ln_eps = 0.f,
                       const void* out_gate = nullptr, void* y2 = nullptr) {
    ConvArgs a;
    Plan p;
    const int st = conv2d_plan(x, gate, y_lo_off, w, bias, residual, y, d, w_lo, x_split, out_scale, status, ln_g, ln_b, ln_eps, &a, &p, out_gate);
    return st != VIP_OK ? st : launch(p, a, d->groups, (hipStream_t)stream, (f16*)y2);
}

static int kernel_query(const char* who, bool variant, const vip_conv_desc* d, int has_residual, int has_gate, int has_w_lo, char* out,
                        size_t cap, bool out_gate = false) {
    VIP_REQUIRE(d && out && cap > 0, VIP_ERR_BAD_ARG, "%s: null pointer", who);
    static const char dummy[16] = {0};
    ConvArgs a;
    Plan p;
    const int st = conv2d_plan(dummy, has_gate ? dummy : nullptr, 0, dummy, nullptr, has_residual ? dummy : nullptr, const_cast<char*>(dummy), d,
                               has_w_lo ? dummy : nullptr, false, 1.f, nullptr, nullptr, nullptr, 0.f, &a, &p, out_gate ? dummy : nullptr);
    if (st != VIP_OK) return st;
    static const char* const kernel[] = {"pw_gemm_kernel",    "rows_gemm_kernel", "gemm8p_kernel",           "pwx_kernel",
                                         "pwk_direct_kernel", "pwk_gemm_kernel",  "pwk_gemm_kernel(im2col)", "conv_igemm_kernel"};
    if (!variant) {
        snprintf(out, cap, "%s", p.family == PWX && p.ln ? "pwx_ln_kernel" : kernel[p.family]);
        return VIP_OK;
    }
    switch (p.family) {
        case PW_GEMM: snprintf(out, cap, "pw_gemm<KS=%d%s> %d x %d%s", p.ks, p.hilo ? ",hilo" : "", p.n_chunks, p.nb_ch, p.mode >= 7 ? " ogate" : ""); break;
        case ROWS_GEMM: snprintf(out, cap, "rows_gemm%s", p.xsplit ? "<xsplit>" : ""); break;
        case GEMM8P: snprintf(out, cap, "gemm8p<%s> %d x %d", p.pipe ? "pipe" : "basic", p.m_blocks, p.n_blocks); break;
        case PWX: snprintf(out, cap, "%s<%d,%d>", p.ln ? "pwx_ln" : "pwx", p.ksc, p.pt); break;
        case PWK_DIRECT:
            if (p.pf2) snprintf(out, cap, "pwk_direct2<%d>", p.ng);
            else snprintf(out, cap, "pwk_direct<%d%s> PT=%d%s", p.ng, p.gated ? ",gated" : "", p.pt, p.mode >= 7 ? " ogate" : "");
            break;
        case PWK_GEMM: snprintf(out, cap, "pwk_gemm<%d,%d> %d x %d", p.ng, p.wn, p.m_blocks, p.n_blocks); break;
        case IM2COL: snprintf(out, cap, "im2col<%d>", p.ng); break;
        case CONV_IGEMM: snprintf(out, cap, "conv_igemm<%d,%d>", p.bm, p.bn); break;
    }
    return VIP_OK;
}

#if VIP_GEMM_H2
extern "C" int vip_conv2d_nhwc_h2(const void* x, const void* w, const float* bias, const void* residual, void* y, const vip_conv_desc* d,
                                  float out_scale, int* status, void* stream) {
    VIP_REQUIRE(out_scale > 0.f, VIP_ERR_BAD_ARG, "vip_conv2d_nhwc_h2: out_scale must be positive");
    return conv2d_impl(x, nullptr, 0, w, bias, residual, y, d, stream, nullptr, false, out_scale, status);
}

extern "C" int vip_conv2d_gated_nhwc_h2(const void* x, const void* gate, const void* w, const float* bias, const void* residual, void* y,
                                        const vip_conv_desc* d, float out_scale, int* status, void* stream) {
    VIP_REQUIRE(gate, VIP_ERR_BAD_ARG, "vip_conv2d_gated_nhwc_h2: null gate");
    VIP_REQUIRE(out_scale > 0.f, VIP_ERR_BAD_ARG, "vip_conv2d_gated_nhwc_h2: out_scale must be positive");
    VIP_REQUIRE(d && d->cin_off == 0 && d->ldx == d->Cin, VIP_ERR_UNSUPPORTED,
                "vip_conv2d_gated_nhwc_h2: the gate indexes the whole input channel axis (cin_off = 0, ldx = Cin)");
    return conv2d_impl(x, gate, 0, w, bias, residual, y, d, stream, nullptr, false, out_scale, status);
}

extern "C" int vip_conv2d_kernel_name_h2(const vip_conv_desc* d, int has_residual, char* name, size_t cap) {
    return kernel_query("vip_conv2d_kernel_name_h2", false, d, has_residual, 0, 0, name, cap);
}

extern "C" int vip_conv2d_kernel_variant_h2(const vip_conv_desc* d, int has_residual, char* variant, size_t cap) {
    return kernel_query("vip_conv2d_kernel_variant_h2", true, d, has_residual, 0, 0, variant, cap);
}
#else
extern "C" int vip_conv2d_nhwc_f16(const void* x, const void* w, const float* bias, const void* residual, void* y,
                                   const vip_conv_desc* d, void* stream) {
    return conv2d_impl(x, nullptr, 0, w, bias, residual, y, d, stream);
}

extern "C" int vip_conv2d_gated_nhwc_f16(const void* x, const void* gate, const void* w, const float* bias,
                                         const void* residual, void* y, const vip_conv_desc* d, void* stream) {
    VIP_REQUIRE(gate, VIP_ERR_BAD_ARG, "vip_conv2d_gated_nhwc_f16: null gate");
    VIP_REQUIRE(d && d->cin_off == 0 && d->ldx == d->Cin, VIP_ERR_UNSUPPORTED,
                "vip_conv2d_gated_nhwc_f16: the gate indexes the whole input channel axis (cin_off = 0, ldx = Cin)");
    return conv2d_impl(x, gate, 0, w, bias, residual, y, d, stream);
}

extern "C" int vip_conv2d_hilo_nhwc_f16(const void* x, const void* w_hi, const void* w_lo, const float* bias,
                                        const void* residual, void* y, const vip_conv_desc* d, void* stream) {
    VIP_REQUIRE(w_lo, VIP_ERR_BAD_ARG, "vip_conv2d_hilo_nhwc_f16: null w_lo");
    return conv2d_impl(x, nullptr, 0, w_hi, bias, residual, y, d, stream, w_lo);
}

extern "C" int vip_conv2d_out_gated_nhwc_f16(const void* x, const void* w, const void* w_lo, const float* bias, const void* out_gate,
                                             const void* residual, void* y, const vip_conv_desc* d, void* stream) {
    VIP_REQUIRE(out_gate && residual, VIP_ERR_BAD_ARG, "vip_conv2d_out_gated_nhwc_f16: null gate or residual");
    return conv2d_impl(x, nullptr, 0, w, bias, residual, y, d, stream, w_lo, false, 1.f, nullptr, nullptr, nullptr, 0.f, out_gate);
}

extern "C" int vip_conv2d_out_gated_variant(const vip_conv_desc* d, int has_w_lo, char* variant, size_t cap) {
    return kernel_query("vip_conv2d_out_gated_variant", true, d, 1, 0, has_w_lo, variant, cap, true);
}

extern "C" int vip_conv2d_out_gated2_nhwc_f16(const void* x, const void* w, const void* w_lo, const float* bias, const void* out_gate,
                                              const void* residual, void* y, void* y2, int act2, const vip_conv_desc* d, void* stream) {
    VIP_REQUIRE(out_gate && residual && y2, VIP_ERR_BAD_ARG, "vip_conv2d_out_gated2_nhwc_f16: null gate, residual or second output");
    VIP_REQUIRE(act2 == VIP_ACT_SILU, VIP_ERR_UNSUPPORTED, "vip_conv2d_out_gated2_nhwc_f16: act2=%d (the second output is built for SiLU)", act2);
    return conv2d_impl(x, nullptr, 0, w, bias, residual, y, d, stream, w_lo, false, 1.f, nullptr, nullptr, nullptr, 0.f, out_gate, y2);
}

extern "C" int vip_conv2d_out_gated2_variant(const vip_conv_desc* d, int has_w_lo, int act2, char* variant, size_t cap) {
    VIP_REQUIRE(act2 == VIP_ACT_SILU, VIP_ERR_UNSUPPORTED, "vip_conv2d_out_gated2_variant: act2=%d (the second output is built for SiLU)", act2);
    const int st = kernel_query("vip_conv2d_out_gated2_variant", true, d, 1, 0, has_w_lo, variant, cap, true);
    if (st != VIP_OK) return st;
    const size_t n = strlen(variant);
    if (n + 4 <= cap) memcpy(variant + n, " y2", 4);
    return VIP_OK;
}

extern "C" int vip_conv2d_kernel_name(const vip_conv_desc* d, int has_residual, int has_gate, int has_w_lo, char* name,
                                      size_t cap) {
    return kernel_query("vip_conv2d_kernel_name", false, d, has_residual, has_gate, has_w_lo, name, cap);
}

extern "C" int vip_conv2d_kernel_variant(const vip_conv_desc* d, int has_residual, int has_gate, int has_w_lo, char* variant,
                                         size_t cap) {
    return kernel_query("vip_conv2d_kernel_variant", true, d, has_residual, has_gate, has_w_lo, variant, cap);
}

static vip_conv_desc gemm_desc(int M, int N, int K, int lda, int ldw, int ldc, int ldr, int act_pre, int act_post) {
    vip_conv_desc d;
    d.B = M; d.H = 1; d.W = 1; d.Cin = K; d.Cout = N; d.kh = d.kw = 1; d.sh = d.sw = 1; d.pt = d.pl = 0;
    d.Ho = d.Wo = 1; d.groups = 1; d.ldx = lda; d.cin_off = 0; d.ldy = ldc; d.cout_off = 0; d.ldr = ldr;
    d.res_off = 0; d.ldw = ldw; d.act_pre = act_pre; d.act_post = act_post;
    return d;
}

extern "C" int vip_gemm_bias_act_f16(const void* A, const void* W, const float* bias, const void* residual,
                                     void* C, int M, int N, int K, int lda, int ldw, int ldc, int ldr,
                                     int act_pre, int act_post, void* stream) {
    const vip_conv_desc d = gemm_desc(M, N, K, lda, ldw, ldc, ldr, act_pre, act_post);
    return vip_conv2d_nhwc_f16(A, W, bias, residual, C, &d, stream);
}

extern "C" int vip_ln_gemm_supported(int M, int K, int N, int act) {
    if (M < 16384 || N < 256 || N % 8 != 0 || K % 8 != 0 || K <= 64 || K > 384 || (unsigned)act > 4u) return 0;
    const char* all = getenv("VIP_LN_GEMM_ALL");
    if (all && atoi(all)) return 1;
    if (M < 65536 && N > 512) return 0;
    return 1;
}

extern "C" int vip_ln_gemm_bias_act_f16(const void* A, const float* ln_gamma, const float* ln_beta, float ln_eps, const void* W,
                                        const float* bias, const void* residual, void* C, int M, int N, int K, int lda, int ldw,
                                        int ldc, int ldr, int act_pre, int act_post, void* stream) {
    VIP_REQUIRE(ln_gamma && ln_beta, VIP_ERR_BAD_ARG, "vip_ln_gemm_bias_act_f16: null LayerNorm parameters");
    VIP_REQUIRE(ln_eps > 0.f, VIP_ERR_BAD_ARG, "vip_ln_gemm_bias_act_f16: eps must be positive");
    const vip_conv_desc d = gemm_desc(M, N, K, lda, ldw, ldc, ldr, act_pre, act_post);
    return conv2d_impl(A, nullptr, 0, W, bias, residual, C, &d, stream, nullptr, false, 1.f, nullptr, ln_gamma, ln_beta, ln_eps);
}

extern "C" int vip_gemm_split_f16(const void* A, const void* W, const float* bias, void* C, int M, int N, int K, int lda,
                                  int ldw, int act, void* stream) {
    VIP_REQUIRE(M > 0 && M <= 256, VIP_ERR_UNSUPPORTED, "vip_gemm_split_f16: M=%d (1..256 rows)", M);
    const vip_conv_desc d = gemm_desc(M, N, K, lda, ldw, 2 * N, 0, act, VIP_ACT_NONE);
    return conv2d_impl(A, nullptr, N, W, bias, nullptr, C, &d, stream);
}

extern "C" int vip_gemm_split2_hilo_f16(const void* A, const void* W, const void* W_lo, const float* bias, void* C, int M, int N, int K,
                                        int ldw, int act, void* stream) {
    VIP_REQUIRE(W_lo, VIP_ERR_BAD_ARG, "vip_gemm_split2_hilo_f16: null W_lo");
    VIP_REQUIRE(M > 0 && M <= 256, VIP_ERR_UNSUPPORTED, "vip_gemm_split2_hilo_f16: M=%d (1..256 rows)", M);
    VIP_REQUIRE(K % 8 == 0, VIP_ERR_ALIGNMENT, "vip_gemm_split2_hilo_f16: K must be a multiple of 8");
    const vip_conv_desc d = gemm_desc(M, N, K, 2 * K, ldw, 2 * N, 0, act, VIP_ACT_NONE);
    return conv2d_impl(A, nullptr, N, W, bias, nullptr, C, &d, stream, W_lo, true);
}

extern "C" int vip_gemm_split2_f16(const void* A, const void* W, const float* bias, void* C, int M, int N, int K, int ldw, int act,
                                   void* stream) {
    VIP_REQUIRE(M > 0 && M <= 256, VIP_ERR_UNSUPPORTED, "vip_gemm_split2_f16: M=%d (1..256 rows)", M);
    VIP_REQUIRE(K % 8 == 0, VIP_ERR_ALIGNMENT, "vip_gemm_split2_f16: K must be a multiple of 8");
    const vip_conv_desc d = gemm_desc(M, N, K, 2 * K, ldw, 2 * N, 0, act, VIP_ACT_NONE);
    return conv2d_impl(A, nullptr, N, W, bias, nullptr, C, &d, stream, nullptr, true);
}
#endif
```

### vip-cup-2022_amd/gcvit.py

```python
from typing import Dict

import torch

from . import ops
from .cam import CamMixin, HeadSpec
from .pipeline import keras_predict
from .synth import ParamGen

NAME2CONFIG = {
    "gcvit_xxtiny": dict(window_size=(7, 7, 14, 7), dim=64, depths=(2, 2, 6, 2), num_heads=(2, 4, 8, 16), mlp_ratio=3.0),
    "gcvit_xtiny": dict(window_size=(7, 7, 14, 7), dim=64, depths=(3, 4, 6, 5), num_heads=(2, 4, 8, 16), mlp_ratio=3.0),
    "gcvit_tiny": dict(window_size=(7, 7, 14, 7), dim=64, depths=(3, 4, 19, 5), num_heads=(2, 4, 8, 16), mlp_ratio=3.0),
    "gcvit_small": dict(window_size=(7, 7, 14, 7), dim=96, depths=(3, 4, 19, 5), num_heads=(3, 6, 12, 24), mlp_ratio=2.0,
                        layer_scale=1e-5),
    "gcvit_base": dict(window_size=(7, 7, 14, 7), dim=128, depths=(3, 4, 19, 5), num_heads=(4, 8, 16, 32), mlp_ratio=2.0,
                       layer_scale=1e-5),
}
KEEP_DIMS = [(False, False, False), (False, False), (True,), (True,)]
LN_EPS = 1e-5
PAD1 = (1, 1, 1, 1)


def synth_params(cfg: Dict, seed: int = 1002, classes: int = 1) -> Dict[str, torch.Tensor]:
    g = ParamGen(seed)
# ... 47 lines not shown
        self.fc0 = ops.make_dense_weight(p[f"{name}/conv/2/fc/0/kernel"], None, dev)
        self.fc2 = ops.make_dense_weight(p[f"{name}/conv/2/fc/2/kernel"], None, dev)
        self.pw = ops.make_conv_weight(p[f"{name}/conv/3/kernel"], None, device=dev)

    def __call__(self, x):
        y, s = ops.dwconv2d_se(x, self.dw, None, 3, 1, PAD1, "gelu", self.fc0, self.fc2, "gelu", "sigmoid")
        return ops.conv2d(y, self.pw, residual=x, gate=s)


class _LN:
    def __init__(self, p, name, dev):
        self.g = p[f"{name}/gamma"].to(dev, torch.float32).contiguous()
        self.b = p[f"{name}/beta"].to(dev, torch.float32).contiguous()

    def __call__(self, x):
        return ops.layernorm(x, self.g, self.b, LN_EPS)


class _ReduceSize:

    def __init__(self, p, name, dev):
        self.n1 = _LN(p, f"{name}/norm1", dev)
        self.n2 = _LN(p, f"{name}/norm2", dev)
        self.branch = _ConvBranch(p, name, dev)
        self.red = ops.make_conv_weight(p[f"{name}/reduction/kernel"], None, device=dev)

    def __call__(self, x, stride=2):
        x = self.branch(self.n1(x))
        return self.n2(ops.conv2d(x, self.red, stride=stride, pad=PAD1))


class _Block:

    def __init__(self, p, name, ws, heads, global_query, dev):
        self.ws, self.heads, self.global_query = ws, heads, global_query
        self.n1 = _LN(p, f"{name}/norm1", dev)
        self.n2 = _LN(p, f"{name}/norm2", dev)
        self.qkv = ops.make_dense_weight(p[f"{name}/attn/qkv/kernel"], p[f"{name}/attn/qkv/bias"], dev)
        g1 = p.get(f"{name}/gamma1")
        g2 = p.get(f"{name}/gamma2")

        def scaled(kernel, bias, g):
            return (kernel, bias) if g is None else (kernel * g[None, :], bias * g)
        self.proj = ops.make_dense_weight(*scaled(p[f"{name}/attn/proj/kernel"], p[f"{name}/attn/proj/bias"], g1), dev)
        self.table = p[f"{name}/attn/relative_position_bias_table"].to(dev, torch.float32).contiguous()
        self.fc1 = ops.make_dense_weight(p[f"{name}/mlp/fc1/kernel"], p[f"{name}/mlp/fc1/bias"], dev)
        self.fc2 = ops.make_dense_weight(*scaled(p[f"{name}/mlp/fc2/kernel"], p[f"{name}/mlp/fc2/bias"], g2), dev)

    def __call__(self, x, q_global):
        C = x.shape[-1]
        hd = C // self.heads
        x = ops.gcvit_attn_block(x, q_global if self.global_query else None, (self.n1.g, self.n1.b, LN_EPS), self.qkv, self.proj,
                                 self.table, self.heads, self.ws, hd ** -0.5)
        return ops.mlp(x, self.fc1, self.fc2, act="gelu", residual=x, ln=(self.n2.g, self.n2.b, LN_EPS))


@keras_predict
class GCViT(CamMixin):
    def __init__(self, params: Dict[str, torch.Tensor], window_size, dim, depths, num_heads, mlp_ratio=3.0,
                 layer_scale=None, classes: int = 1, device="cuda", first_strides: int = 2, head_act: str = "default"):
        p, dev = params, device
        self.first_strides = first_strides
        self.head_act = head_act
        self.cfg = dict(window_size=window_size, dim=dim, depths=depths, num_heads=num_heads, mlp_ratio=mlp_ratio)
        self.classes = classes
        self.stem = ops.make_conv_weight(p["patch_embed/proj/kernel"], p["patch_embed/proj/bias"], device=dev,
                                         pad_cin_to=8)
        self.stem_down = _ReduceSize(p, "patch_embed/conv_down", dev)
        self.levels = []
        n = len(depths)
        for i in range(n):
            lv = {
                "ws": window_size[i],
                "qgen": [(_ConvBranch(p, f"levels/{i}/q_global_gen/to_q_global/{k}", dev), kd)
                         for k, kd in enumerate(KEEP_DIMS[i])],
                "blocks": [_Block(p, f"levels/{i}/blocks/{j}", window_size[i], num_heads[i], bool(j % 2), dev)
                           for j in range(depths[i])],
                "down": _ReduceSize(p, f"levels/{i}/downsample", dev) if i < n - 1 else None,
            }
            self.levels.append(lv)
        self.norm = _LN(p, "norm", dev)
        self.head_w = p["head/kernel"].t().contiguous().to(dev, torch.float32)
        self.head_b = p["head/bias"].to(dev, torch.float32)

    def _level(self, x, lv):
        ws = lv["ws"]
        B, H, W, C = x.shape
        ph, pw = (ws - H % ws) % ws, (ws - W % ws) % ws
        if ph or pw:
            x = ops.pool2d(x, 1, 1, (ph // 2, ph // 2 + ph % 2, pw // 2, pw // 2 + pw % 2), ops.POOL_MAX_ZEROPAD)
        qg = x
        for branch, keep_dim in lv["qgen"]:
            qg = branch(qg)
            if not keep_dim:
                qg = ops.pool2d(qg, 3, 2, PAD1, ops.POOL_MAX_ZEROPAD)
        qg = qg.reshape(B, ws * ws, C)
        for blk in lv["blocks"]:
            x = blk(x, qg)
        if ph or pw:
            x = ops.pool2d(x, 1, 1, (0, 0, 0, 0), ops.POOL_MAX_ZEROPAD, out_hw=(H, W))
        if lv["down"] is not None:
            x = lv["down"](x)
        return x

    def features(self, x, collect=None):
        assert x.shape[-1] == 8
        y = ops.conv2d(x, self.stem, stride=2, pad=PAD1)
        y = self.stem_down(y, stride=self.first_strides)
        if collect is not None:
            collect.append(y)
        for lv in self.levels:
            y = self._level(y, lv)
            if collect is not None:
                collect.append(y)
        return self.norm(y)

    def head_spec(self) -> HeadSpec:
        return HeadSpec(self.head_w, self.head_b, None, getattr(self, "head_act", "default"))

    def logits(self, x):
        return ops.gap_dense_f32(self.features(x), self.head_w, self.head_b)

    def predict(self, x):
        z = self.logits(x)
        return ops.head_prob(z, getattr(self, "head_act", "default"))


def GCViTTiny(params, classes=1, device="cuda", first_strides=2, head_act="default"):
    return GCViT(params, **NAME2CONFIG["gcvit_tiny"], classes=classes, device=device, first_strides=first_strides, head_act=head_act)
```

### vip-cup-2022_amd/ops.py

```python
import ctypes as C
import math
import os
from dataclasses import dataclass
from typing import Optional

import numpy as np
import torch

from . import _abi


def _env_flag(name: str, default: bool) -> bool:
    v = os.environ.get(name)
    return default if v is None else (v != "0" if default else v == "1")


def _env_int(name: str, default: int) -> int:
    return int(os.environ.get(name, default))


PRECISION = os.environ.get("VIP_PRECISION", "fast")
STRICT_GEMM = os.environ.get("VIP_STRICT_GEMM", "bf16x3")
_LN_GEMM = _env_flag("VIP_LN_GEMM", True)
_MLP_H2_FUSED = _env_flag("VIP_MLP_H2_FUSED", True)
_SE_H2_FUSED = _env_flag("VIP_SE_H2_FUSED", True)
_H2_GATED = _env_flag("VIP_H2_GATED", True)
_DW_H2_LDS = _env_int("VIP_DW_H2_LDS", 3)
_SE_TAIL = _env_flag("VIP_SE_TAIL", True)
_DW_SE_FUSED = _env_flag("VIP_DW_SE_POOL", True)
_GCVIT_BLOCK_FUSED = _env_flag("VIP_GCVIT_BLOCK_FUSED", True)
_GCVIT_BLOCK14 = _env_flag("VIP_GCVIT_BLOCK14", False)


def hilo_enabled() -> bool:
    return _env_flag("VIP_HILO", True)


def mbconv_fused() -> bool:
    return _env_flag("VIP_MBCONV_FUSED", False)


def offset_calibration() -> bool:
    return _env_flag("VIP_OFFSET_CALIBRATION", False)


ACT = {None: 0, "none": 0, "linear": 0, "relu": 1, "silu": 2, "swish": 2, "gelu": 3, "sigmoid": 4}


_PROF = None


def set_profiler(p):
    global _PROF
    _PROF = p


def _act(a):
    if isinstance(a, int):
        return a
    return ACT[a]


def _stream():
    return C.c_void_p(torch.cuda.current_stream().cuda_stream)


def _p(t: Optional[torch.Tensor]):
    return C.c_void_p(0 if t is None else t.data_ptr())


def _chk16(t: torch.Tensor, name: str):
    if t.dtype != torch.float16 or not t.is_cuda or not t.is_contiguous():
        raise _abi.VipError(f"{name}: expected a contiguous CUDA float16 tensor, got {t.dtype} {t.device} "
                            f"contiguous={t.is_contiguous()}")


def _chk32(t: torch.Tensor, name: str):
    if t.dtype != torch.float32 or not t.is_cuda or not t.is_contiguous():
        raise _abi.VipError(f"{name}: expected a contiguous CUDA float32 tensor (strict path), got {t.dtype} {t.device} "
                            f"contiguous={t.is_contiguous()}")


def _is32(t: torch.Tensor, name: str) -> bool:
    if t.dtype == torch.float32:
        _chk32(t, name)
        return True
    _chk16(t, name)
    return False


PACKED = torch.int32


def _chkp(t: torch.Tensor, name: str):
    if t.dtype != PACKED or not t.is_cuda or not t.is_contiguous() or t.shape[-1] % 8:
        raise _abi.VipError(f"{name}: expected a contiguous CUDA packed-strict (int32 carrier) tensor with C % 8 == 0, got {t.dtype} "
                            f"{t.device} {tuple(t.shape)} contiguous={t.is_contiguous()}")


def _kind(t: torch.Tensor, name: str) -> str:
    if t.dtype == PACKED:
        _chkp(t, name)
        return "h2"
    return "s32" if _is32(t, name) else "f16"


# ... 37 lines not shown
    "layernorm": (_ALL_KINDS, True),
    "pool2d_nhwc": (_ALL_KINDS, True),
    "global_avgpool": (_ALL_KINDS, True),
    "mul": (_ALL_KINDS, True),
    "vit_tokens": (_ALL_KINDS, True),
    "mhsa_fwd": (_ALL_KINDS, True),
    "dwconv2d_nhwc": (_ALL_KINDS, True),
    "window_attn_fwd": (_ALL_KINDS, True),
    "cam": ({"f16": "f32", "s32": "s32", "h2": "h2"}, False),
    "scale_add_act": (_STRICT_KINDS, True),
    "radix_combine": (_STRICT_KINDS, True),
    "gap_ln_dense": (_STRICT_KINDS, False),
}


def _launch_kind(base: str, kind: str, *args, prof=None):
    suffix, status = _KIND_OPS[base]
    _launch(f"vip_{base}_{suffix[kind]}", *args, status=status and kind == "h2", prof=prof)


def pack_h2(x: torch.Tensor) -> torch.Tensor:
    _chk32(x, "pack_h2.x")
    assert x.shape[-1] % 8 == 0, x.shape
    out = torch.empty(x.shape, dtype=PACKED, device=x.device)
    _launch("vip_pack_h2", _p(x), _p(out), x.numel(), status=True)
    return out


def unpack_h2(x: torch.Tensor) -> torch.Tensor:
    _chkp(x, "unpack_h2.x")
    out = torch.empty(x.shape, dtype=torch.float32, device=x.device)
    _launch("vip_unpack_h2", _p(x), _p(out), x.numel())
    return out


PRECISIONS = ("fast", "strict", "f32")


class precision:

    def __init__(self, mode: str):
        if mode not in PRECISIONS:
            raise ValueError(f"precision {mode!r}: expected one of {PRECISIONS}")
        self.mode = mode

    def __enter__(self):
        global PRECISION
        self._old, PRECISION = PRECISION, self.mode
        return self

    def __exit__(self, *exc):
        global PRECISION
        PRECISION = self._old
        return False


def to_act(t: torch.Tensor, device="cuda", dtype: Optional[torch.dtype] = None) -> torch.Tensor:
    dtype = dtype or act_dtype()
    if dtype == PACKED:
        return pack_h2(t.detach().to(device=device, dtype=torch.float32).contiguous())
    return t.detach().to(device=device, dtype=dtype).contiguous()


def act_dtype(mode: Optional[str] = None) -> torch.dtype:
    return {"fast": torch.float16, "strict": PACKED, "f32": torch.float32}[mode or PRECISION]


@dataclass
class ConvWeight:
    w: torch.Tensor
    bias: Optional[torch.Tensor]
    kh: int
    kw: int
    cin_g: int
    cout: int
    groups: int = 1
    alg_cin_g: int = 0
    err: Optional[torch.Tensor] = None
    w_lo: Optional[torch.Tensor] = None
    exact: Optional["ConvWeight"] = None
    w_bf3: Optional[torch.Tensor] = None
    h2_scale: float = 0.0
    fold: Optional[tuple] = None

    @property
    def cin(self):
        return self.cin_g * self.groups

    @property
    def strict(self):
        return self.w.dtype == torch.float32

    @property
    def kind(self):
        return "h2" if self.h2_scale > 0 else ("s32" if self.strict else "f16")

    @property
    def ldw(self):
        return self.w.shape[1]


KEEP_ROUNDING_ERROR = False
_CALIB = False
_UNFUSED = False
_EXACT = False
_EXACT_REG: list = []


class calibration:

    def __enter__(self):
        global _CALIB, _UNFUSED
        self._old = (_CALIB, _UNFUSED)
        _CALIB = _UNFUSED = True
        return self

    def __exit__(self, *exc):
        global _CALIB, _UNFUSED
        _CALIB, _UNFUSED = self._old
        if not offset_calibration():
            drop_exact_weights()
        return False


class unfused:

    def __enter__(self):
        global _UNFUSED
        self._old = _UNFUSED
        _UNFUSED = True
        return self

    def __exit__(self, *exc):
        global _UNFUSED
        _UNFUSED = self._old
        return False


class exact_weights:

    def __enter__(self):
        global _UNFUSED, _EXACT
        self._old = (_UNFUSED, _EXACT)
        _UNFUSED = _EXACT = True
        return self

    def __exit__(self, *exc):
        global _UNFUSED, _EXACT
        _UNFUSED, _EXACT = self._old
        return False


def drop_exact_weights():
    for cw in _EXACT_REG:
        cw.exact = None
    _EXACT_REG.clear()


def _exact_operands(x: torch.Tensor, cw: "ConvWeight", cin_off: int = 0):
    xs = x[..., cin_off:cin_off + cw.cin]
    lead = xs.shape[:-1]
    xg = xs.reshape(*lead, cw.groups, cw.cin_g)
    return torch.cat([xg, xg], -1).reshape(*lead, 2 * cw.cin).contiguous(), cw.exact, 0


def _bias_correct(cw: "ConvWeight", x_eff: torch.Tensor):
# ... 361 lines not shown
    out, d = _conv_front("h2", x, cw, stride, pad, act, act_post, residual, out, cin_off, cout_off)
    B = d.B
    per_img = 4 * max(d.H * d.W * d.ldx, d.Ho * d.Wo * d.ldy, d.Ho * d.Wo * d.ldr)
    bmax = max(1, (_H2_SPAN_MAX - 1) // per_img)

    def prof():
        return _conv_prof("h2:" + ("pwk_direct_kernel" if gate is not None else conv_kernel_name_h2(d, residual is not None) or "unsupported"),
                          d, cw, residual, 4.0, 2.0)
    for b0 in range(0, B, bmax):
        b1 = min(B, b0 + bmax)
        d.B = b1 - b0
        rs = None if residual is None else residual[b0:b1]
        tail = (_p(cw.w), _p(cw.bias), _p(rs), _p(out[b0:b1]), C.byref(d), 1.0 / cw.h2_scale)
        if gate is not None:
            _launch("vip_conv2d_gated_nhwc_h2", _p(x[b0:b1]), _p(gate[b0:b1]), *tail, status=True, prof=prof)
        else:
            _launch("vip_conv2d_nhwc_h2", _p(x[b0:b1]), *tail, status=True, prof=prof)
    return out


def _conv2d_s32(x, cw: ConvWeight, stride, pad, act, act_post, residual, out, cin_off, cout_off, gate):
    if gate is not None:
        assert gate.shape == (x.shape[0], cw.cin) and x.shape[3] == cw.cin and cin_off == 0, (gate.shape, x.shape, cw.cin)
        x = scale_add_act(x, gate, None, None)
    out, d = _conv_front("s32", x, cw, stride, pad, act, act_post, residual, out, cin_off, cout_off)
    split = STRICT_GEMM in ("bf16x3", "bf16x2") and cw.w_bf3 is not None

    def prof():
        return _conv_prof("sconv6_kernel" if split else "sconv_kernel", d, cw, residual, 4.0, 4.0)
    tail = (_p(cw.bias), _p(residual), _p(out), C.byref(d))
    if split:
        _launch("vip_conv2d_nhwc_s32x2" if STRICT_GEMM == "bf16x2" else "vip_conv2d_nhwc_s32x", _p(x), _p(cw.w_bf3), cw.w_bf3.shape[2], *tail,
                prof=prof)
    else:
        _launch("vip_conv2d_nhwc_s32", _p(x), _p(cw.w), *tail, prof=prof)
    return out


_CONV_STRICT = {"s32": _conv2d_s32, "h2": _conv2d_h2}


def _rows_out(x, cw: ConvWeight, residual, name: str):
    K = x.shape[-1]
    out = torch.empty((*x.shape[:-1], cw.cout), dtype=torch.float16, device=x.device)
    if residual is not None:
        _chk16(residual, name)
        assert residual.shape == out.shape
    return x.numel() // K, K, out, 0 if residual is None else cw.cout


def dense(x: torch.Tensor, cw: ConvWeight, act=None, act_post=None, residual: Optional[torch.Tensor] = None):
    kind = _kind(x, "dense.x")
    if kind != "f16":
        if kind != cw.kind:
            raise _abi.VipError(f"dense: {kind} activations with {cw.kind} weights - build the model and its input in the same precision")
        lead, K = x.shape[:-1], x.shape[-1]
        r4 = None if residual is None else residual.reshape(-1, 1, 1, cw.cout)
        return _CONV_STRICT[kind](x.reshape(-1, 1, 1, K), cw, 1, (0, 0, 0, 0), act, act_post, r4, None, 0, 0, None).reshape(*lead, cw.cout)
    if _CALIB and cw.err is not None:
        _bias_correct(cw, x)
    if _EXACT and cw.exact is not None:
        x, cw, _ = _exact_operands(x, cw)
    M, K, out, ldr = _rows_out(x, cw, residual, "dense.residual")

    def prof():
        d = _abi.ConvDesc(B=M, H=1, W=1, Cin=K, Cout=cw.cout, kh=1, kw=1, sh=1, sw=1, pt=0, pl=0, Ho=1, Wo=1, groups=1, ldx=K,
                          cin_off=0, ldy=cw.cout, cout_off=0, ldr=ldr, res_off=0, ldw=cw.ldw, act_pre=_act(act),
                          act_post=_act(act_post))
        return (conv_kernel_name(d, residual is not None) or "unsupported", 2.0 * M * cw.cout * K,
                2.0 * (M * K + M * cw.cout * (2 if residual is not None else 1) + cw.w.numel()),
                f"M={M} N={cw.cout} K={K} dense{' res' if residual is not None else ''} act={act}")
    _launch("vip_gemm_bias_act_f16", _p(x), _p(cw.w), _p(cw.bias), _p(residual), _p(out), M, cw.cout, K, K, cw.ldw, cw.cout, ldr,
            _act(act), _act(act_post), prof=prof)
    return out


def ln_gemm_fused(x: torch.Tensor, cw: ConvWeight, act=None, act_post=None, residual: Optional[torch.Tensor] = None) -> bool:
    K = x.shape[-1]
    return bool(_LN_GEMM and not (_UNFUSED or _CALIB or _EXACT) and x.dtype == torch.float16 and x.is_contiguous() and cw.kind == "f16"
                and _pointwise(cw) and cw.cin == K and 2 * x.numel() < 0xFFFF0000 - 2 * K and _epilogue_ok(act, act_post, residual)
                and _abi.lib().vip_ln_gemm_supported(x.numel() // K, K, cw.cout, _act(act)))


def ln_dense(x: torch.Tensor, ln, cw: ConvWeight, act=None, act_post=None, residual: Optional[torch.Tensor] = None):
    g, b, eps = _ln_args(ln)
    if not ln_gemm_fused(x, cw, act, act_post, residual):
        return dense(layernorm(x, g, b, eps), cw, act=act, act_post=act_post, residual=residual)
    M, K, out, ldr = _rows_out(x, cw, residual, "ln_dense.residual")
    _launch("vip_ln_gemm_bias_act_f16", _p(x), _p(g), _p(b), eps, _p(cw.w), _p(cw.bias), _p(residual), _p(out), M, cw.cout, K, K, cw.ldw,
            cw.cout, ldr, _act(act), _act(act_post),
            prof=lambda: ("pwx_ln_kernel", 2.0 * M * cw.cout * K,
                          2.0 * (M * K + M * cw.cout * (2 if residual is not None else 1) + cw.w.numel()) + 8.0 * K,
                          f"M={M} N={cw.cout} K={K} ln+dense{' res' if residual is not None else ''} act={act}"))
    return out


def mlp(x: torch.Tensor, fc1: ConvWeight, fc2: ConvWeight, act="gelu", residual: Optional[torch.Tensor] = None, ln=None):
    kind = _kind(x, "mlp.x")
    C_ = x.shape[-1]
    M = x.numel() // C_
    hid = fc1.cout
    g, b, eps = _ln_args(ln)
    ldr = C_ if residual is not None else 0
    if kind == "f16":
        fused = (not _UNFUSED and fc2.cout == C_ and fc1.groups == 1 and fc2.groups == 1 and x.is_contiguous()
                 and _abi.lib().vip_mlp_fused_supported(M, C_, hid, _act(act)))
    else:
        fused = (kind == "h2" and _MLP_H2_FUSED and not _UNFUSED and fc1.kind == fc2.kind == "h2" and fc2.cout == C_ and fc1.cin == C_
                 and fc2.cin == hid and _pointwise(fc1) and _pointwise(fc2) and x.is_contiguous() and 4 * x.numel() < _H2_SPAN_MAX
                 and _abi.lib().vip_mlp_fused_supported_h2(M, C_, hid, _act(act)))
    if not fused:
        if ln is not None and kind == "f16":
            return dense(ln_dense(x, ln, fc1, act=act), fc2, residual=residual)
        if ln is not None:
            x = layernorm(x, g, b, eps)
        return dense(dense(x, fc1, act=act), fc2, residual=residual)
    out = torch.empty_like(x)
    if residual is not None:
        _chk_kind(residual, kind, "mlp.residual")
        assert residual.shape == out.shape
    if kind == "h2":
        _launch("vip_mlp_fused_h2", _p(x), _p(g), _p(b), eps, _p(fc1.w), _p(fc1.bias), 1.0 / fc1.h2_scale, _p(fc2.w), _p(fc2.bias),
                1.0 / fc2.h2_scale, _p(residual), _p(out), M, C_, hid, C_, fc1.ldw, fc2.ldw, C_, ldr, _act(act), status=True,
                prof=lambda: ("h2:mlp_h2_kernel", 4.0 * M * C_ * hid,
                              4.0 * M * C_ * (3 if residual is not None else 2) + 2.0 * (fc1.w.numel() + fc2.w.numel()),
                              f"M={M} C={C_} hidden={hid}"))
    else:
        _launch("vip_mlp_fused_f16", _p(x), _p(g), _p(b), eps, _p(fc1.w), _p(fc1.bias), _p(fc2.w), _p(fc2.bias), _p(residual), _p(out),
                M, C_, hid, C_, fc1.ldw, fc2.ldw, C_, ldr, _act(act),
                prof=lambda: ("mlp_fused_kernel" if C_ <= 96 else "mlp_stream_kernel", 4.0 * M * C_ * hid,
                              2.0 * (M * C_ * (3 if residual is not None else 2) + fc1.w.numel() + fc2.w.numel())))
    return out


def se_gate(x: torch.Tensor, fc1: ConvWeight, fc2: ConvWeight, act1, act2="sigmoid", split: bool = True) -> torch.Tensor:
    kind = _kind(x, "se_gate.x")
    if kind != "f16":
        B, Cc = x.shape[0], x.shape[-1]
        if kind == "h2" and _SE_H2_FUSED and fc1.kind == fc2.kind == "h2" and _se_chain_ok(fc1, fc2, Cc) and x.dim() == 4:
            out = torch.empty((B, fc2.cout), dtype=PACKED, device=x.device)
            _launch("vip_se_gate_h2", _p(x), _p(fc1.w), _p(fc1.bias), 1.0 / fc1.h2_scale, _p(fc2.w), _p(fc2.bias), 1.0 / fc2.h2_scale,
                    _p(out), B, x.shape[1] * x.shape[2], Cc, Cc, fc1.cout, fc1.ldw, fc2.cout, fc2.ldw, _act(act1), _act(act2), status=True)
            return out
        return dense(dense(global_avgpool(x), fc1, act=act1), fc2, act=act2)
    B, H, W, Cc = x.shape
    assert _pointwise(fc1) and _pointwise(fc2)
    assert fc1.cin == Cc and fc2.cin == fc1.cout, (fc1.cin, Cc, fc2.cin, fc1.cout)
    if _UNFUSED or not _se_chain_ok(fc1, fc2, Cc):
        g = dense_split(dense_split(global_avgpool(x, split=True), fc1, act=act1), fc2, act=act2)
        return g if split else g[:, 0].contiguous()
    out = torch.empty((B, 2, fc2.cout) if split else (B, fc2.cout), dtype=torch.float16, device=x.device)
    tail = (_p(fc1.bias), _p(fc2.w), _p(fc2.bias), _p(out), B, H * W, Cc, Cc, fc1.cout, fc1.ldw, fc2.cout, fc2.ldw, _act(act1), _act(act2),
            int(split))
    if fc1.w_lo is not None:
        _launch("vip_se_gate_hilo_f16", _p(x), _p(fc1.w), _p(fc1.w_lo), *tail)
    else:
        _launch("vip_se_gate_f16", _p(x), _p(fc1.w), *tail)
    return out


def dense_split(x: torch.Tensor, cw: ConvWeight, act=None) -> torch.Tensor:
    if _kind(x, "dense_split.x") != "f16":
        return dense(x, cw, act=act)
    split_in = x.dim() == 3
    assert x.dim() == 2 or (split_in and x.shape[1] == 2), x.shape
    if _CALIB and cw.err is not None:
        _bias_correct(cw, x.float().sum(1) if split_in else x)
    if _EXACT and cw.exact is not None:
        x, cw, _ = _exact_operands(x, cw)
# ... 465 lines not shown
```

### vip-cup-2022_amd/tfimm_models.py

```python
from dataclasses import dataclass
from typing import Dict, Tuple

import torch

from . import _abi, ops
from .cam import VIT_REASON, CamMixin, HeadSpec
from .pipeline import keras_predict
from .synth import ParamGen

LN_EPS = 1e-6


class _LN:
    def __init__(self, p, name, dev):
        self.g = p[f"{name}/gamma"].to(dev, torch.float32).contiguous()
        self.b = p[f"{name}/beta"].to(dev, torch.float32).contiguous()

    def __call__(self, x):
        return ops.layernorm(x, self.g, self.b, LN_EPS)


@dataclass
class ViTConfig:
    name: str
# ... 42 lines not shown
    if tuple(src_grid) == tuple(tgt_grid):
        return pos_embed
    pe = pos_embed.detach().cpu().to(torch.float32).numpy()
    D = pe.shape[-1]
    src = pe[nb_tokens:].reshape(src_grid[0], src_grid[1], D)
    iy, wy = _tf_bicubic_taps(tgt_grid[0], src_grid[0])
    ix, wx = _tf_bicubic_taps(tgt_grid[1], src_grid[1])
    rows = None
    for t in range(4):
        term = src[:, ix[:, t], :] * wx[None, :, t, None]
        rows = term if rows is None else rows + term
    out = None
    for t in range(4):
        term = rows[iy[:, t], :, :] * wy[:, t, None, None]
        out = term if out is None else out + term
    out = np.concatenate([pe[:nb_tokens], out.reshape(tgt_grid[0] * tgt_grid[1], D).astype(np.float32)], 0)
    return torch.from_numpy(out)


def variant(cfg, overrides: Dict):
    import dataclasses
    if not overrides:
        return cfg
    known = {f.name for f in dataclasses.fields(cfg)}
    bad = set(overrides) - known
    if bad:
        raise ValueError(f"{cfg.name}: unknown config fields {sorted(bad)}")
    return dataclasses.replace(cfg, **overrides)


VIT_CONFIGS = {
    "vit_tiny_patch16_224": ViTConfig("vit_tiny_patch16_224", embed_dim=192, nb_heads=3),
    "vit_small_patch16_224": ViTConfig("vit_small_patch16_224", embed_dim=384, nb_heads=6),
    "vit_base_patch16_224": ViTConfig("vit_base_patch16_224", embed_dim=768, nb_heads=12),
}


def vit_synth_params(cfg: ViTConfig, seed: int) -> Dict[str, torch.Tensor]:
    g = ParamGen(seed)
    D, ps = cfg.embed_dim, cfg.patch_size
    g.conv("patch_embed/proj", ps, ps, 3, D, bias=True, gain=1.0)
    g.raw("cls_token", g._n((1, 1, D), 0.5))
    g.raw("pos_embed", g._n((1, cfg.nb_patches + 1, D), 0.5))
    hid = int(D * cfg.mlp_ratio)
    for j in range(cfg.nb_blocks):
        b = f"blocks/{j}"
        g.ln(f"{b}/norm1", D)
        g.dense(f"{b}/attn/qkv", D, 3 * D, bias=cfg.qkv_bias)
        g.dense(f"{b}/attn/proj", D, D, gain=0.25)
        g.ln(f"{b}/norm2", D)
        g.dense(f"{b}/mlp/fc1", D, hid, gain=2.0)
        g.dense(f"{b}/mlp/fc2", hid, D, gain=0.25)
    g.ln("norm", D)
    g.dense("head", D, cfg.nb_classes)
    return g.p


@keras_predict
class ViT:
    def __init__(self, params: Dict[str, torch.Tensor], cfg: ViTConfig, device="cuda"):
        p, dev = params, device
        self.cfg = cfg
        D = cfg.embed_dim
        assert D // cfg.nb_heads == 64, "vip_mhsa_fwd_f16 implements head_dim 64"
        self.patch = ops.make_conv_weight(p["patch_embed/proj/kernel"], p["patch_embed/proj/bias"], device=dev, pad_cin_to=8)
        self.cls = ops.to_act(p["cls_token"].reshape(D), dev)
        self.pos = ops.to_act(p["pos_embed"].reshape(-1, D), dev)
        self._pos32 = p["pos_embed"].reshape(-1, D).to(torch.float32)
        self._pos_by_grid = {tuple(cfg.grid_size): self.pos}
        self._act_dtype, self._dev = ops.act_dtype(), dev
        self.blocks = []
        for j in range(cfg.nb_blocks):
            b = f"blocks/{j}"
            qkv_bias = p.get(f"{b}/attn/qkv/bias")
            self.blocks.append(dict(
                n1=_LN(p, f"{b}/norm1", dev), n2=_LN(p, f"{b}/norm2", dev),
                qkv=ops.make_dense_weight(p[f"{b}/attn/qkv/kernel"], qkv_bias, dev),
                proj=ops.make_dense_weight(p[f"{b}/attn/proj/kernel"], p[f"{b}/attn/proj/bias"], dev),
                fc1=ops.make_dense_weight(p[f"{b}/mlp/fc1/kernel"], p[f"{b}/mlp/fc1/bias"], dev),
                fc2=ops.make_dense_weight(p[f"{b}/mlp/fc2/kernel"], p[f"{b}/mlp/fc2/bias"], dev)))
        self.norm = _LN(p, "norm", dev)
        self.head_w = p["head/kernel"].t().contiguous().to(dev, torch.float32)
        self.head_b = p["head/bias"].to(dev, torch.float32)

    def features(self, x, collect=None):
        cfg = self.cfg
        assert x.shape[-1] == 8
        if not cfg.interpolate_input and tuple(x.shape[1:3]) != tuple(cfg.input_size):
            raise ValueError(f"{cfg.name}: interpolate_input=False (vit.py:58): the input must be {cfg.input_size}, got {tuple(x.shape[1:3])}")
        B = x.shape[0]
        ps = cfg.patch_size
        pe = ops.conv2d(x, self.patch, stride=ps)
        grid = (pe.shape[1], pe.shape[2])
        if grid not in self._pos_by_grid:
            pos = interpolate_pos_embeddings(self._pos32, cfg.grid_size, grid, nb_tokens=1)
            self._pos_by_grid[grid] = ops.to_act(pos, self._dev, self._act_dtype)
        t = ops.vit_tokens(pe.reshape(B, grid[0] * grid[1], cfg.embed_dim), self.cls, self._pos_by_grid[grid])
        scale = (cfg.embed_dim // cfg.nb_heads) ** -0.5
        for blk in self.blocks:
            qkv = ops.ln_dense(t, (blk["n1"].g, blk["n1"].b, LN_EPS), blk["qkv"])
            att = ops.mhsa(qkv, cfg.nb_heads, scale)
            t = ops.dense(att, blk["proj"], residual=t)
            t = ops.mlp(t, blk["fc1"], blk["fc2"], act="gelu", residual=t, ln=(blk["n2"].g, blk["n2"].b, LN_EPS))
            if collect is not None:
                collect.append(t)
        return self.norm(t)

    cam_supported = False
    cam_unsupported_reason = VIT_REASON

    def cam(self, x, target="score"):
        raise _abi.VipError(f"{self.cfg.name}: no evidence map - {VIT_REASON}")

    def predict_with_cam(self, x, target="score"):
        raise _abi.VipError(f"{self.cfg.name}: no evidence map - {VIT_REASON}")

    def logits(self, x):
        t = self.features(x)
        return ops.cls_dense_f32(t, self.head_w, self.head_b)

    def predict(self, x):
        z = self.logits(x)
        return ops.head_prob(z, getattr(self, "head_act", "default"))


@dataclass
class ConvNeXtConfig:
    name: str
    patch_size: int = 4
    first_down: int = 1
    embed_dim: Tuple = (96, 192, 384, 768)
    nb_blocks: Tuple = (3, 3, 9, 3)
    mlp_ratio: float = 4.0
    nb_classes: int = 1


CONVNEXT_CONFIGS = {
    "convnext_tiny_in22k": ConvNeXtConfig("convnext_tiny_in22k"),
    "convnext_small_in22k": ConvNeXtConfig("convnext_small_in22k", nb_blocks=(3, 3, 27, 3)),
    "convnext_base_in22k": ConvNeXtConfig("convnext_base_in22k", embed_dim=(128, 256, 512, 1024), nb_blocks=(3, 3, 27, 3)),
    "convnext_large_in22ft1k": ConvNeXtConfig("convnext_large_in22ft1k", embed_dim=(192, 384, 768, 1536), nb_blocks=(3, 3, 27, 3)),
    "convnext_base_384_in22ft1k": ConvNeXtConfig("convnext_base_384_in22ft1k", embed_dim=(128, 256, 512, 1024), nb_blocks=(3, 3, 27, 3)),
    "convnext_large_384_in22ft1k": ConvNeXtConfig("convnext_large_384_in22ft1k", embed_dim=(192, 384, 768, 1536), nb_blocks=(3, 3, 27, 3)),
}


def convnext_synth_params(cfg: ConvNeXtConfig, seed: int) -> Dict[str, torch.Tensor]:
    g = ParamGen(seed)
    g.conv("stem/0", cfg.patch_size, cfg.patch_size, 3, cfg.embed_dim[0], bias=True, gain=1.0)
    g.ln("stem/1", cfg.embed_dim[0])
    cprev = cfg.embed_dim[0]
    for j, (c, nb) in enumerate(zip(cfg.embed_dim, cfg.nb_blocks)):
        if j > 0:
            g.ln(f"stages/{j}/downsample/0", cprev)
            g.conv(f"stages/{j}/downsample/1", 2, 2, cprev, c, bias=True, gain=1.0)
        hid = int(cfg.mlp_ratio * c)
        for i in range(nb):
            b = f"stages/{j}/blocks/{i}"
            g.dwconv(f"{b}/conv_dw", 7, c, bias=True, gain=1.0)
            g.ln(f"{b}/norm", c)
            g.dense(f"{b}/mlp/fc1", c, hid, gain=2.0)
            g.dense(f"{b}/mlp/fc2", hid, c)
            g.raw(f"{b}/gamma", g._u((c,), 0.1, 0.4))
        cprev = c
    g.ln("head/norm", cprev)
    g.dense("head/fc", cprev, cfg.nb_classes)
# ... 60 lines not shown
```

Measured before the change: 4915 images/sec.

## Fold LayerNorm into following GEMM weights and apply stats in epilogue

Adds an LN-folded dense path for the layers where the existing fused LN+GEMM kernel is not taken. The LayerNorm gamma is folded into the weights and beta into the bias. Per-row mean and variance are accumulated inside the pointwise direct GEMM kernel from the operand fragments it already loads, and are applied in the epilogue as (acc - mu*s)*rstd + b'. This removes the separate LayerNorm launch and its activation read/write for the ViT and GCViT qkv/fc1 layers within certain size ranges. In exchange it adds fp16 statistics arithmetic, extra epilogue loads, different rounding, and precomputed folded weights.

```diff
diff --git a/include/vipcup_hip.h b/include/vipcup_hip.h
--- a/include/vipcup_hip.h
+++ b/include/vipcup_hip.h
@@ -62,6 +62,12 @@
 int vip_ln_gemm_bias_act_f16(const void* A, const float* ln_gamma, const float* ln_beta, float ln_eps, const void* W,
                              const float* bias, const void* residual, void* C, int M, int N, int K, int lda, int ldw,
                              int ldc, int ldr, int act_pre, int act_post, void* stream);
+
+int vip_lnfold_gemm_supported(int M, int K, int N, int act);
+int vip_lnfold_gemm_bias_act_f16(const void* A, const void* Wf, const float* s, const float* bias_f, float ln_eps, const void* residual,
+                                 void* C, int M, int N, int K, int lda, int ldw, int ldc, int ldr, int act_pre, int act_post,
+                                 void* stream);
+int vip_lnfold_gemm_variant(int M, int N, int K, int act_pre, int act_post, int has_residual, int has_gate, char* variant, size_t cap);
 
 int vip_gemm_split_f16(const void* A, const void* W, const float* bias, void* C, int M, int N, int K, int lda,
                        int ldw, int act, void* stream);
diff --git a/vip-cup-2022_amd/_abi.py b/vip-cup-2022_amd/_abi.py
--- a/vip-cup-2022_amd/_abi.py
+++ b/vip-cup-2022_amd/_abi.py
@@ -72,6 +72,9 @@
     "vip_gemm_bias_act_f16": (_i, [_vp, _vp, _vp, _vp, _vp] + [_i] * 9 + [_vp]),
     "vip_ln_gemm_supported": (_i, [_i, _i, _i, _i]),
     "vip_ln_gemm_bias_act_f16": (_i, [_vp, _vp, _vp, _f] + [_vp] * 4 + [_i] * 9 + [_vp]),
+    "vip_lnfold_gemm_supported": (_i, [_i, _i, _i, _i]),
+    "vip_lnfold_gemm_bias_act_f16": (_i, [_vp, _vp, _vp, _vp, _f, _vp, _vp] + [_i] * 9 + [_vp]),
+    "vip_lnfold_gemm_variant": (_i, [_i] * 7 + [C.c_char_p, _sz]),
     "vip_mlp_fused_supported": (_i, [_i, _i, _i, _i]),
     "vip_mlp_fused_plan": (_i, [_i] * 4 + [C.POINTER(_i)] * 2),
     "vip_mlp_fused_f16": (_i, [_vp, _vp, _vp, _f] + [_vp] * 6 + [_i] * 9 + [_vp]),
diff --git a/vip-cup-2022_amd/csrc/conv_igemm.hip b/vip-cup-2022_amd/csrc/conv_igemm.hip
--- a/vip-cup-2022_amd/csrc/conv_igemm.hip
+++ b/vip-cup-2022_amd/csrc/conv_igemm.hip
@@ -63,6 +63,7 @@
     int ng, pt, wn, ks, ksc, bm, bn;
     bool gated, hilo, ln, xsplit, pipe;
     bool pf2;
+    bool lnf;
     int m_blocks, n_blocks;
     int n_chunks, nb_ch, lds_stride;
 };
@@ -421,11 +422,18 @@
     return img0;
 }
 
-template <int PT, int ACT, bool RES, bool POST_RELU, bool OGATE = false, bool Y2 = false>
+template <int PT>
+struct LnFoldEpi {
+    float mu[PT], rstd[PT];
+    __amdgpu_buffer_rsrc_t rb_s, rb_b;
+};
+
+template <int PT, int ACT, bool RES, bool POST_RELU, bool OGATE = false, bool Y2 = false, bool LNF = false>
 __device__ __forceinline__ void pw_epilogue(const ConvArgs& a, f32x4 (&acc)[PT][4], int m_base, int n_first,
                                             const __amdgpu_buffer_rsrc_t& rb_res, const __amdgpu_buffer_rsrc_t& rb_y, GateLds gl = GateLds{},
-                                            const __amdgpu_buffer_rsrc_t* rb_y2 = nullptr) {
+                                            const __amdgpu_buffer_rsrc_t* rb_y2 = nullptr, const LnFoldEpi<PT>* lf = nullptr) {
     constexpr unsigned OOB = 0xFFFFFFF0u;
+    static_assert(!(LNF && (H2 || OGATE)), "the folded LayerNorm: fp16 storage, no output gate");
     if constexpr (H2) {
 #pragma unroll
         for (int p = 0; p < PT; ++p) {
@@ -443,6 +451,18 @@
     }
     static_assert(!(OGATE && H2), "the output gate is carried by the fp16-storage build only");
     static_assert(OGATE || !Y2, "the second output belongs to the output-gated epilogue");
+    f32x4 lf_s[LNF ? 2 : 1][2], lf_b[LNF ? 2 : 1][2];
+    if constexpr (LNF) {
+#pragma unroll
+        for (int h = 0; h < 2; ++h)
+#pragma unroll
+            for (int q = 0; q < 2; ++q) {
+                const int n = n_first + h * 32 + q * 4;
+                const unsigned off = n < a.Cout_g ? (unsigned)(n * 4) : OOB;
+                lf_s[h][q] = __builtin_bit_cast(f32x4, __builtin_amdgcn_raw_buffer_load_b128(lf->rb_s, off, 0, 0));
+                lf_b[h][q] = __builtin_bit_cast(f32x4, __builtin_amdgcn_raw_buffer_load_b128(lf->rb_b, off, 0, 0));
+            }
+    }
 #pragma unroll
     for (int p = 0; p < PT; ++p) {
         const int m = m_base + p * 16;
@@ -465,7 +485,12 @@
 #pragma unroll
             for (int j = 0; j < 8; j += 2) {
                 const f32x4 av = acc[p][h * 2 + (j >> 2)];
-                f32x2 t = vip_act2<ACT>((f32x2){av[j & 3], av[(j & 3) + 1]});
+                f32x2 v = {av[j & 3], av[(j & 3) + 1]};
+                if constexpr (LNF) {
+                    const f32x4 sq = lf_s[h][j >> 2], bq = lf_b[h][j >> 2];
+                    v = (v - lf->mu[p] * (f32x2){sq[j & 3], sq[(j & 3) + 1]}) * lf->rstd[p] + (f32x2){bq[j & 3], bq[(j & 3) + 1]};
+                }
+                f32x2 t = vip_act2<ACT>(v);
                 if constexpr (OGATE) {
                     const f32x4 gq = j < 4 ? g0 : g1;
                     t = t * (f32x2){gq[j & 3], gq[(j & 3) + 1]};
@@ -688,9 +713,12 @@
     return vip_launch_status("vip_conv2d_out_gated2_nhwc_f16(pw)");
 }
 
-template <int NG, bool GATED, int PT = 4, bool OG2 = false>
+template <int NG, bool GATED, int PTL = 4, bool OG2 = false>
 __global__ __launch_bounds__(256, 2) void pwk_direct_kernel(std::conditional_t<OG2, ConvArgs2, ConvArgs> a, int mode) {
+    constexpr bool LNF = PTL < 0;
+    constexpr int PT = LNF ? -PTL : PTL;
     static_assert(!(OG2 && (GATED || H2)), "the second output: fp16 storage, no input gate");
+    static_assert(!(LNF && (GATED || OG2 || H2)), "the folded LayerNorm: fp16 storage, no input gate, no output gate");
     constexpr int NB = 64 * NG, ROWB = 160;
     constexpr int STAGE = NB * ROWB;
     constexpr int W_IT = NB / 32;
@@ -814,7 +842,7 @@
                 const f32x4 bv = __builtin_bit_cast(
                     f32x4, __builtin_amdgcn_raw_buffer_load_b128(rb_bias, n < a.Cout_g ? (unsigned)(n * 4) : OOB, 0, 0));
 #pragma unroll
-                for (int p = 0; p < PT; ++p) acc[g][p][nt] = bv;
+                for (int p = 0; p < PT; ++p) acc[g][p][nt] = LNF ? (f32x4){0.f, 0.f, 0.f, 0.f} : bv;
             }
     }
 
@@ -825,6 +853,28 @@
     store_w(0);
     __syncthreads();
 
+    f16x2 ln_c[LNF ? PT : 1];
+    float ln_s1[LNF ? PT : 1], ln_s2[LNF ? PT : 1];
+    if constexpr (LNF) {
+#pragma unroll
+        for (int p = 0; p < PT; ++p) {
+            ln_c[p] = (f16x2){xf[0][p].e[0], xf[0][p].e[0]};
+            ln_s1[p] = ln_s2[p] = 0.f;
+        }
+    }
+    auto ln_stats = [&](int ks, int p) {
+        if constexpr (LNF) {
+            const f16x2 one = {(f16)1.f, (f16)1.f};
+            const unsigned xw[4] = {xf[ks][p].u.x, xf[ks][p].u.y, xf[ks][p].u.z, xf[ks][p].u.w};
+#pragma unroll
+            for (int e = 0; e < 4; ++e) {
+                const f16x2 d = __builtin_bit_cast(f16x2, xw[e]) - ln_c[p];
+                ln_s2[p] = __builtin_amdgcn_fdot2(d, d, ln_s2[p], false);
+                ln_s1[p] = __builtin_amdgcn_fdot2(d, one, ln_s1[p], false);
+            }
+        }
+    };
+
     auto compute = [&](int buf, int ks) {
         const char* ws = smem + buf * STAGE + l15 * ROWB + lq * 16 + ks * 64;
 #pragma unroll
@@ -854,10 +904,12 @@
             for (int nt = 0; nt < 4; ++nt) wf[nt].u = *reinterpret_cast<const uint4*>(ws + (g * 64 + nt * 16) * ROWB);
             if (VIP_MFMA_PRIO) __builtin_amdgcn_s_setprio(1);
 #pragma unroll
-            for (int nt = 0; nt < 4; ++nt)
+            for (int nt = 0; nt < 4; ++nt) {
 #pragma unroll
                 for (int p = 0; p < PT; ++p)
                     acc[g][p][nt] = __builtin_amdgcn_mfma_f32_16x16x32_f16(wf[nt].h, xf[ks][p].h, acc[g][p][nt], 0, 0, 0);
+                if (g == 0 && nt < PT) ln_stats(ks, nt);
+            }
             if (VIP_MFMA_PRIO) __builtin_amdgcn_s_setprio(0);
         }
     };
@@ -898,7 +950,26 @@
     asm volatile("" : "+v"(m_base), "+v"(n_lane));
     GateLds gl{};
 #if !VIP_GEMM_H2
-    if constexpr (!GATED) {
+    LnFoldEpi<PT> lf;
+    if constexpr (LNF) {
+        const float n = 0.25f * (float)a.K, rn = 1.f / n;
+#pragma unroll
+        for (int p = 0; p < PT; ++p) {
+            float mean = (float)ln_c[p].x + ln_s1[p] * rn;
+            float m2 = fmaxf(ln_s2[p] - ln_s1[p] * ln_s1[p] * rn, 0.f);
+            float mo = __shfl_xor(mean, 16, 64), qo = __shfl_xor(m2, 16, 64), dl = mean - mo;
+            m2 = (m2 + qo) + dl * dl * (0.5f * n);
+            mean = 0.5f * (mean + mo);
+            mo = __shfl_xor(mean, 32, 64), qo = __shfl_xor(m2, 32, 64), dl = mean - mo;
+            m2 = (m2 + qo) + dl * dl * n;
+            mean = 0.5f * (mean + mo);
+            lf.mu[p] = mean;
+            lf.rstd[p] = rsqrtf(m2 / (float)a.K + a.ln_eps);
+        }
+        lf.rb_s = __builtin_amdgcn_make_buffer_rsrc((void*)a.ln_g, 0, (unsigned)(a.bias_elems * 4), 0x00020000);
+        lf.rb_b = rb_bias;
+    }
+    if constexpr (!GATED && !LNF) {
         if (mode >= 7) {
             float* g_lds = reinterpret_cast<float*>(smem);
             const int img0 = stage_out_gate(a, g_lds, NB, mb * (64 * PT), 64 * PT, n0, NB, (int)threadIdx.x, 256);
@@ -915,6 +986,19 @@
             const __amdgpu_buffer_rsrc_t rb_y2 = __builtin_amdgcn_make_buffer_rsrc((void*)a.y2, 0, (unsigned)a.y_span_bytes, 0x00020000);
             if (mode == 8) pw_epilogue<PT, VIP_ACT_NONE, true, true, true, true>(a, acc[G_], m_base, n_first, rb_res, rb_y, gl, &rb_y2);
             else pw_epilogue<PT, VIP_ACT_NONE, true, false, true, true>(a, acc[G_], m_base, n_first, rb_res, rb_y, gl, &rb_y2);
+            return;
+        }
+        if constexpr (LNF) {
+            const GateLds ng{};
+            switch (mode) {
+                case 1: pw_epilogue<PT, VIP_ACT_RELU, false, false, false, false, true>(a, acc[G_], m_base, n_first, rb_res, rb_y, ng, nullptr, &lf); break;
+                case 2: pw_epilogue<PT, VIP_ACT_SILU, false, false, false, false, true>(a, acc[G_], m_base, n_first, rb_res, rb_y, ng, nullptr, &lf); break;
+                case 3: pw_epilogue<PT, VIP_ACT_GELU, false, false, false, false, true>(a, acc[G_], m_base, n_first, rb_res, rb_y, ng, nullptr, &lf); break;
+                case 4: pw_epilogue<PT, VIP_ACT_SIGMOID, false, false, false, false, true>(a, acc[G_], m_base, n_first, rb_res, rb_y, ng, nullptr, &lf); break;
+                case 5: pw_epilogue<PT, VIP_ACT_NONE, true, false, false, false, true>(a, acc[G_], m_base, n_first, rb_res, rb_y, ng, nullptr, &lf); break;
+                case 6: pw_epilogue<PT, VIP_ACT_NONE, true, true, false, false, true>(a, acc[G_], m_base, n_first, rb_res, rb_y, ng, nullptr, &lf); break;
+                default: pw_epilogue<PT, VIP_ACT_NONE, false, false, false, false, true>(a, acc[G_], m_base, n_first, rb_res, rb_y, ng, nullptr, &lf); break;
+            }
             return;
         }
 #endif
@@ -935,6 +1019,11 @@
     epi(std::integral_constant<int, 0>{});
     if constexpr (NG > 1) epi(std::integral_constant<int, 1>{});
 }
+
+#if !VIP_GEMM_H2
+template <int NG, int PT>
+constexpr auto pwk_lnfold_kernel = pwk_direct_kernel<NG, false, -PT>;
+#endif
 
 
 template <int KSC, int PT, bool LN>
@@ -1556,6 +1645,13 @@
 template <int NG>
 int launch_pwk_direct(const ConvArgs& a, const Plan& p, hipStream_t s) {
     auto go = [&](auto kernel) { hipLaunchKernelGGL(kernel, dim3((unsigned)(a.m_blocks * a.n_blocks)), dim3(256), 0, s, a, p.mode); };
+#if !VIP_GEMM_H2
+    if (p.lnf) {
+        if (p.gated || p.pf2 || p.mode < 0 || p.mode > 6) return (int)VIP_ERR_UNSUPPORTED;
+        p.pt == 1 ? go(pwk_lnfold_kernel<NG, 1>) : go(pwk_lnfold_kernel<NG, 4>);
+        return vip_launch_status("vip_lnfold_gemm_bias_act_f16(pwk-direct)");
+    }
+#endif
     if (p.pt == 1) p.gated ? go(pwk_direct_kernel<NG, true, 1>) : go(pwk_direct_kernel<NG, false, 1>);
 #if VIP_BUILD_EXPERIMENTS
     else if (p.pf2) go(pwk_direct2_kernel<NG>);
@@ -1942,7 +2038,7 @@
 
 static int conv2d_plan(const void* x, const void* gate, int y_lo_off, const void* w, const float* bias, const void* residual, void* y,
                        const vip_conv_desc* d, const void* w_lo, bool x_split, float out_scale, int* status, const float* ln_g,
-                       const float* ln_b, float ln_eps, ConvArgs* args, Plan* p, const void* out_gate = nullptr) {
+                       const float* ln_b, float ln_eps, ConvArgs* args, Plan* p, const void* out_gate = nullptr, bool ln_fold = false) {
     VIP_REQUIRE(x && w && y && d, VIP_ERR_BAD_ARG, "vip_conv2d_nhwc_f16: null pointer");
     VIP_REQUIRE(d->B > 0 && d->H > 0 && d->W > 0 && d->Cin > 0 && d->Cout > 0 && d->kh > 0 && d->kw > 0 &&
                     d->sh > 0 && d->sw > 0 && d->Ho > 0 && d->Wo > 0 && d->groups > 0 && d->pt >= 0 && d->pl >= 0,
@@ -1993,6 +2089,24 @@
     a.ogate = (const f16*)out_gate;
     a.ogate_elems = 0;
     a.hw_magic = a.gate_hw > 1 ? (unsigned)((1L << 32) / a.gate_hw) : 0xFFFFFFFFu;
+#if !VIP_GEMM_H2
+    if (ln_fold) {
+        VIP_REQUIRE(ln_g && !ln_b && bias && !gate && !out_gate && !w_lo && !y_lo_off && !x_split && d->groups == 1 && d->kh == 1 && d->kw == 1 &&
+                        d->sh == 1 && d->sw == 1 && d->pt == 0 && d->pl == 0 && d->Ho == d->H && d->Wo == d->W && d->cin_off == 0 &&
+                        vip_lnfold_gemm_supported((int)M, a.K, cout_g, d->act_pre),
+                    VIP_ERR_UNSUPPORTED, "vip_lnfold_gemm_bias_act_f16: M=%ld K=%d N=%d act=%d/%d not taken (vip_lnfold_gemm_supported: "
+                    "K %% 64 == 0, 64 < K < 768, no gate)", M, a.K, cout_g, d->act_pre, d->act_post);
+        a.ln_g = nullptr;
+        const int st = plan(a, d, x_split, p);
+        a.ln_g = ln_g;
+        if (st != VIP_OK) return st;
+        VIP_REQUIRE(p->family == PWK_DIRECT && !p->gated && !p->pf2 && p->mode >= 0 && p->mode <= 6, VIP_ERR_UNSUPPORTED,
+                    "vip_lnfold_gemm_bias_act_f16: M=%ld K=%d N=%d: the plain call does not select pwk_direct_kernel with an (activation) or "
+                    "(residual [+ReLU]) epilogue", M, a.K, cout_g);
+        p->lnf = true;
+        return VIP_OK;
+    }
+#endif
     if (!out_gate) return plan(a, d, x_split, p);
     VIP_REQUIRE(!H2 && residual && !gate && !y_lo_off && !x_split && !ln_g && d->groups == 1 && d->cout_off == 0 && d->act_pre == VIP_ACT_NONE &&
                     (d->act_post == VIP_ACT_NONE || d->act_post == VIP_ACT_RELU) && 4L * d->B * d->Cout < 0xFFFFFFF0L,
@@ -2013,21 +2127,24 @@
 static int conv2d_impl(const void* x, const void* gate, int y_lo_off, const void* w, const float* bias, const void* residual, void* y,
                        const vip_conv_desc* d, void* stream, const void* w_lo = nullptr, bool x_split = false, float out_scale = 1.f,
                        int* status = nullptr, const float* ln_g = nullptr, const float* ln_b = nullptr, float ln_eps = 0.f,
-                       const void* out_gate = nullptr, void* y2 = nullptr) {
+                       const void* out_gate = nullptr, void* y2 = nullptr, bool ln_fold = false) {
     ConvArgs a;
     Plan p;
-    const int st = conv2d_plan(x, gate, y_lo_off, w, bias, residual, y, d, w_lo, x_split, out_scale, status, ln_g, ln_b, ln_eps, &a, &p, out_gate);
+    const int st = conv2d_plan(x, gate, y_lo_off, w, bias, residual, y, d, w_lo, x_split, out_scale, status, ln_g, ln_b, ln_eps, &a, &p, out_gate,
+                               ln_fold);
     return st != VIP_OK ? st : launch(p, a, d->groups, (hipStream_t)stream, (f16*)y2);
 }
 
 static int kernel_query(const char* who, bool variant, const vip_conv_desc* d, int has_residual, int has_gate, int has_w_lo, char* out,
-                        size_t cap, bool out_gate = false) {
+                        size_t cap, bool out_gate = false, bool ln_fold = false) {
     VIP_REQUIRE(d && out && cap > 0, VIP_ERR_BAD_ARG, "%s: null pointer", who);
     static const char dummy[16] = {0};
     ConvArgs a;
     Plan p;
-    const int st = conv2d_plan(dummy, has_gate ? dummy : nullptr, 0, dummy, nullptr, has_residual ? dummy : nullptr, const_cast<char*>(dummy), d,
-                               has_w_lo ? dummy : nullptr, false, 1.f, nullptr, nullptr, nullptr, 0.f, &a, &p, out_gate ? dummy : nullptr);
+    const float* fdummy = reinterpret_cast<const float*>(dummy);
+    const int st = conv2d_plan(dummy, has_gate ? dummy : nullptr, 0, dummy, ln_fold ? fdummy : nullptr, has_residual ? dummy : nullptr,
+                               const_cast<char*>(dummy), d, has_w_lo ? dummy : nullptr, false, 1.f, nullptr, ln_fold ? fdummy : nullptr, nullptr,
+                               0.f, &a, &p, out_gate ? dummy : nullptr, ln_fold);
     if (st != VIP_OK) return st;
     static const char* const kernel[] = {"pw_gemm_kernel",    "rows_gemm_kernel", "gemm8p_kernel",           "pwx_kernel",
                                          "pwk_direct_kernel", "pwk_gemm_kernel",  "pwk_gemm_kernel(im2col)", "conv_igemm_kernel"};
@@ -2042,7 +2159,7 @@
         case PWX: snprintf(out, cap, "%s<%d,%d>", p.ln ? "pwx_ln" : "pwx", p.ksc, p.pt); break;
         case PWK_DIRECT:
             if (p.pf2) snprintf(out, cap, "pwk_direct2<%d>", p.ng);
-            else snprintf(out, cap, "pwk_direct<%d%s> PT=%d%s", p.ng, p.gated ? ",gated" : "", p.pt, p.mode >= 7 ? " ogate" : "");
+            else snprintf(out, cap, "pwk_direct<%d%s> PT=%d%s", p.ng, p.gated ? ",gated" : p.lnf ? ",lnfold" : "", p.pt, p.mode >= 7 ? " ogate" : "");
             break;
         case PWK_GEMM: snprintf(out, cap, "pwk_gemm<%d,%d> %d x %d", p.ng, p.wn, p.m_blocks, p.n_blocks); break;
         case IM2COL: snprintf(out, cap, "im2col<%d>", p.ng); break;
@@ -2162,6 +2279,32 @@
     return conv2d_impl(A, nullptr, 0, W, bias, residual, C, &d, stream, nullptr, false, 1.f, nullptr, ln_gamma, ln_beta, ln_eps);
 }
 
+extern "C" int vip_lnfold_gemm_supported(int M, int K, int N, int act) {
+    if (M <= 0 || N <= 0 || N % 8 != 0 || K % 64 != 0 || K <= 64 || K >= 768 || (unsigned)act > 4u) return 0;
+    const char* all = getenv("VIP_LN_FOLD_ALL");
+    if (all && atoi(all)) return 1;
+    if (M < 8192 || M >= 65536 || N <= 512) return 0;
+    if (act == VIP_ACT_GELU && M >= 32768) return 0;
+    return 1;
+}
+
+extern "C" int vip_lnfold_gemm_bias_act_f16(const void* A, const void* Wf, const float* s, const float* bias_f, float ln_eps,
+                                            const void* residual, void* C, int M, int N, int K, int lda, int ldw, int ldc, int ldr,
+                                            int act_pre, int act_post, void* stream) {
+    VIP_REQUIRE(s && bias_f, VIP_ERR_BAD_ARG, "vip_lnfold_gemm_bias_act_f16: null row sums or folded bias");
+    VIP_REQUIRE(ln_eps > 0.f, VIP_ERR_BAD_ARG, "vip_lnfold_gemm_bias_act_f16: eps must be positive");
+    const vip_conv_desc d = gemm_desc(M, N, K, lda, ldw, ldc, ldr, act_pre, act_post);
+    return conv2d_impl(A, nullptr, 0, Wf, bias_f, residual, C, &d, stream, nullptr, false, 1.f, nullptr, s, nullptr, ln_eps, nullptr, nullptr,
+                       true);
+}
+
+extern "C" int vip_lnfold_gemm_variant(int M, int N, int K, int act_pre, int act_post, int has_residual, int has_gate, char* variant,
+                                       size_t cap) {
+    VIP_REQUIRE(M > 0 && N > 0 && K > 0, VIP_ERR_BAD_ARG, "vip_lnfold_gemm_variant: non-positive dimension");
+    const vip_conv_desc d = gemm_desc(M, N, K, K, K, N, has_residual ? N : 0, act_pre, act_post);
+    return kernel_query("vip_lnfold_gemm_variant", true, &d, has_residual, has_gate, 0, variant, cap, false, true);
+}
+
 extern "C" int vip_gemm_split_f16(const void* A, const void* W, const float* bias, void* C, int M, int N, int K, int lda,
                                   int ldw, int act, void* stream) {
     VIP_REQUIRE(M > 0 && M <= 256, VIP_ERR_UNSUPPORTED, "vip_gemm_split_f16: M=%d (1..256 rows)", M);
diff --git a/vip-cup-2022_amd/gcvit.py b/vip-cup-2022_amd/gcvit.py
--- a/vip-cup-2022_amd/gcvit.py
+++ b/vip-cup-2022_amd/gcvit.py
@@ -153,6 +153,14 @@
         self.norm = _LN(p, "norm", dev)
         self.head_w = p["head/kernel"].t().contiguous().to(dev, torch.float32)
         self.head_b = p["head/bias"].to(dev, torch.float32)
+        if not ops.KEEP_ROUNDING_ERROR:
+            self.prepare()
+
+    def prepare(self):
+        for lv in self.levels:
+            for blk in lv["blocks"]:
+                ops.ln_fold_prepare(blk.qkv, (blk.n1.g, blk.n1.b, LN_EPS))
+                ops.ln_fold_prepare(blk.fc1, (blk.n2.g, blk.n2.b, LN_EPS))
 
     def _level(self, x, lv):
         ws = lv["ws"]
diff --git a/vip-cup-2022_amd/ops.py b/vip-cup-2022_amd/ops.py
--- a/vip-cup-2022_amd/ops.py
+++ b/vip-cup-2022_amd/ops.py
@@ -22,6 +22,7 @@
 PRECISION = os.environ.get("VIP_PRECISION", "fast")
 STRICT_GEMM = os.environ.get("VIP_STRICT_GEMM", "bf16x3")
 _LN_GEMM = _env_flag("VIP_LN_GEMM", True)
+_LN_FOLD = _env_flag("VIP_LN_FOLD", True)
 _MLP_H2_FUSED = _env_flag("VIP_MLP_H2_FUSED", True)
 _SE_H2_FUSED = _env_flag("VIP_SE_H2_FUSED", True)
 _H2_GATED = _env_flag("VIP_H2_GATED", True)
@@ -225,6 +226,8 @@
     w_bf3: Optional[torch.Tensor] = None
     h2_scale: float = 0.0
     fold: Optional[tuple] = None
+    ln_s: Optional[torch.Tensor] = None
+    ln_cal: Optional[tuple] = None
 
     @property
     def cin(self):
@@ -752,9 +755,73 @@
                 and _abi.lib().vip_ln_gemm_supported(x.numel() // K, K, cw.cout, _act(act)))
 
 
+def _ln_fold_capable(cw: ConvWeight) -> bool:
+    return bool(cw.kind == "f16" and _pointwise(cw) and cw.w_lo is None and cw.ldw == cw.cin and cw.cin % 64 == 0 and 64 < cw.cin < 768)
+
+
+def ln_fold(cw: ConvWeight, ln) -> ConvWeight:
+    g, b = ln[0], ln[1]
+    cal = cw.ln_cal if (cw.err is None and cw.ln_cal is not None and cw.ln_cal[0] is g) else None
+    tag = ["ln_fold", g, g._version, b, b._version, cw.bias, None if cw.bias is None else cw.bias._version, cal, cw.err]
+    f = cw.fold
+    if f is not None and len(f[0]) == len(tag) and all(a is b_ or (type(a) is int and type(b_) is int and a == b_) for a, b_ in zip(f[0], tag)):
+        return f[1]
+    k, dev = cw.cin, cw.w.device
+    w = cw.w[:, :k].detach().cpu().double()
+    if cw.err is not None:
+        w = w + cw.err[:, :k].detach().cpu().double()
+    g64, b64 = g.detach().cpu().double(), b.detach().cpu().double()
+    wf = cal[2].detach().cpu() if cal is not None else (w * g64).to(torch.float16)
+    wf64 = wf.double()
+    bf = w @ b64
+    if cw.bias is not None:
+        bf = bf + cw.bias.detach().cpu().double()
+    if cal is not None:
+        bf = bf + (w * g64 - wf64) @ cal[1].detach().cpu().double()
+    twin = ConvWeight(w=wf.to(dev).contiguous(), bias=bf.float().to(dev).contiguous(), kh=1, kw=1, cin_g=k, cout=cw.cout, groups=1,
+                      alg_cin_g=cw.alg_cin_g, ln_s=wf64.sum(1).float().to(dev).contiguous())
+    cw.fold = (tag, twin)
+    return twin
+
+
+def ln_fold_prepare(cw: ConvWeight, ln) -> Optional[ConvWeight]:
+    return ln_fold(cw, ln) if (_LN_FOLD and _ln_fold_capable(cw)) else None
+
+
+def _ln_fold_calibrate(x: torch.Tensor, g: torch.Tensor, eps: float, cw: ConvWeight):
+    k = cw.cin
+    xh = layernorm(x, torch.ones_like(g), torch.zeros_like(g), eps)
+    w32 = cw.w[:, :k].double() + cw.err[:, :k].double()
+    cw.ln_cal = (g, xh.reshape(-1, k).float().mean(0), (w32 * g.double()).to(torch.float16).contiguous())
+
+
+def ln_fold_variant(M: int, N: int, K: int, act=None, act_post=None, residual: bool = False, gated: bool = False) -> Optional[str]:
+    buf = C.create_string_buffer(64)
+    st = _abi.lib().vip_lnfold_gemm_variant(M, N, K, _act(act), _act(act_post), int(residual), int(gated), buf, 64)
+    return buf.value.decode() if st == 0 else None
+
+
+def ln_fold_taken(x: torch.Tensor, cw: ConvWeight, act=None, act_post=None, residual: Optional[torch.Tensor] = None) -> bool:
+    K = x.shape[-1]
+    return bool(_LN_FOLD and not (_UNFUSED or _CALIB or _EXACT) and x.dtype == torch.float16 and x.is_contiguous() and cw.cin == K
+                and _ln_fold_capable(cw) and 2 * x.numel() < 0xFFFF0000 - 2 * K and _epilogue_ok(act, act_post, residual)
+                and ln_fold_variant(x.numel() // K, cw.cout, K, act, act_post, residual is not None) is not None)
+
+
 def ln_dense(x: torch.Tensor, ln, cw: ConvWeight, act=None, act_post=None, residual: Optional[torch.Tensor] = None):
     g, b, eps = _ln_args(ln)
     if not ln_gemm_fused(x, cw, act, act_post, residual):
+        if ln_fold_taken(x, cw, act, act_post, residual):
+            tw = ln_fold(cw, ln)
+            M, K, out, ldr = _rows_out(x, cw, residual, "ln_dense.residual")
+            _launch("vip_lnfold_gemm_bias_act_f16", _p(x), _p(tw.w), _p(tw.ln_s), _p(tw.bias), eps, _p(residual), _p(out), M, cw.cout, K, K,
+                    tw.ldw, cw.cout, ldr, _act(act), _act(act_post),
+                    prof=lambda: ("pwk_lnfold_kernel", 2.0 * M * cw.cout * K,
+                                  2.0 * (M * K + M * cw.cout * (2 if residual is not None else 1) + cw.w.numel()) + 8.0 * cw.cout,
+                                  f"M={M} N={cw.cout} K={K} lnfold+dense{' res' if residual is not None else ''} act={act}"))
+            return out
+        if _CALIB and cw.err is not None and x.dtype == torch.float16 and _ln_fold_capable(cw) and cw.cin == x.shape[-1]:
+            _ln_fold_calibrate(x, g, eps, cw)
         return dense(layernorm(x, g, b, eps), cw, act=act, act_post=act_post, residual=residual)
     M, K, out, ldr = _rows_out(x, cw, residual, "ln_dense.residual")
     _launch("vip_ln_gemm_bias_act_f16", _p(x), _p(g), _p(b), eps, _p(cw.w), _p(cw.bias), _p(residual), _p(out), M, cw.cout, K, K, cw.ldw,
diff --git a/vip-cup-2022_amd/tfimm_models.py b/vip-cup-2022_amd/tfimm_models.py
--- a/vip-cup-2022_amd/tfimm_models.py
+++ b/vip-cup-2022_amd/tfimm_models.py
@@ -148,6 +148,13 @@
         self.norm = _LN(p, "norm", dev)
         self.head_w = p["head/kernel"].t().contiguous().to(dev, torch.float32)
         self.head_b = p["head/bias"].to(dev, torch.float32)
+        if not ops.KEEP_ROUNDING_ERROR:
+            self.prepare()
+
+    def prepare(self):
+        for blk in self.blocks:
+            ops.ln_fold_prepare(blk["qkv"], (blk["n1"].g, blk["n1"].b, LN_EPS))
+            ops.ln_fold_prepare(blk["fc1"], (blk["n2"].g, blk["n2"].b, LN_EPS))
 
     def features(self, x, collect=None):
         cfg = self.cfg
```

After: 4934 images/sec, median of 6. About the same (+0.4%).
